# multimodallearning/convexAdam

Measured on AMD Instinct MI355X. Metric: volume-pairs/sec (160x192x224 MIND convex+Adam(80it)), higher is better.
Workload: dtype f32

## Files before the change

### convexadam_amd/_lib.py

```python
import ctypes as C
import os
import threading

import torch

_HERE = os.path.dirname(os.path.abspath(__file__))
LIB_PATH = os.environ.get("CONVEXADAM_HIP_LIB") or os.path.join(_HERE, "csrc", "libconvexadam_hip.so")

ABI_VERSION = 2
CVX_OK, CVX_ERR_INVALID_ARG, CVX_ERR_WORKSPACE, CVX_ERR_LAUNCH, CVX_ERR_UNSUPPORTED = 0, -1, -2, -3, -4


class CvxError(RuntimeError):
    def __init__(self, code, msg):
        super().__init__("libconvexadam_hip error %d: %s" % (code, msg))
        self.code = code


class Smoother(C.Structure):
    _fields_ = [("kind", C.c_int), ("n_boxes", C.c_int), ("box_k", C.c_int * 4), ("gauss_w", C.c_float * 5)]


class CorrOpts(C.Structure):
    _fields_ = [("cost", C.c_int), ("n_box", C.c_int), ("fast", C.c_int), ("f16", C.c_int)]


class PairParams(C.Structure):
    _fields_ = [("H", C.c_int), ("W", C.c_int), ("D", C.c_int), ("mind_r", C.c_int), ("mind_d", C.c_int),
                ("lambda_weight", C.c_float), ("grid_sp", C.c_int), ("disp_hw", C.c_int), ("selected_niter", C.c_int),
                ("selected_smooth", C.c_int), ("grid_sp_adam", C.c_int), ("ic", C.c_int), ("n_feat", C.c_int),
                ("cost_scale", C.c_float), ("cost", C.c_int), ("n_box", C.c_int), ("n_spline_pools", C.c_int), ("corr_fast", C.c_int),
                ("fp16_storage", C.c_int), ("ctx", C.c_void_p), ("adam_fast", C.c_int), ("reserved_", C.c_int * 3)]


_vp, _i, _f, _sz, _i64 = C.c_void_p, C.c_int, C.c_float, C.c_size_t, C.c_int64

SIGNATURES = {
    "cvx_version": (_i, []),
    "cvx_last_error": (C.c_char_p, []),
    "cvx_device_count": (_i, []),
    "cvx_context_create": (_vp, []),
    "cvx_context_destroy": (None, [_vp]),
    "cvx_context_bind": (_vp, [_vp]),
    "cvx_context_set_option": (_i, [_vp, C.c_char_p, C.c_longlong]),
    "cvx_context_get_option": (C.c_longlong, [_vp, C.c_char_p]),
    "cvx_context_set_adam_sqrt_table": (_i, [_vp, _vp, _vp]),
    "cvx_context_set_mind_exp_table": (_i, [_vp, _vp, C.c_uint, C.c_uint, _vp]),
    "cvx_set_adam_sqrt_table": (_i, [_vp]),
    "cvx_set_mind_exp_table": (_i, [_vp, C.c_uint, C.c_uint]),
    "cvx_expf_f32": (_i, [_vp, _vp, _sz, _vp]),
    "cvx_set_option": (_i, [C.c_char_p, C.c_longlong]),
    "cvx_get_option": (C.c_longlong, [C.c_char_p]),
    "cvx_affine_base_host": (None, [_i, _vp]),
    "cvx_disp_mesh_host": (None, [_i, _vp]),
    "cvx_disp_mesh_f32": (_i, [_i, _vp, _vp]),
    "cvx_affine_base_f32": (_i, [_i, _vp, _vp]),
    "cvx_mindssc_workspace_bytes": (_sz, [_i] * 5),
    "cvx_mindssc_f32": (_i, [_vp, _i, _i, _i, _i, _i, _vp, _vp, _sz, _vp]),
    "cvx_mindssc_pooled_scratch_bytes": (_sz, [_i] * 7),
    "cvx_mindssc_pooled_f32": (_i, [_vp, _i, _i, _i, _i, _i, _i, _vp, _i, _vp, _vp, _sz, _vp, _sz, _vp, _vp]),
    "cvx_avgpool_f32": (_i, [_vp, _i, _i, _i, _i, _i, _vp, _vp]),
    "cvx_round_f16_f32": (_i, [_vp, _i64, _vp]),
    "cvx_pack_field_f64": (_i, [_vp, _i, _i, _i, _i, _vp, _vp]),
    "cvx_box_smooth_workspace_bytes": (_sz, [_i] * 5),
    "cvx_box_smooth_f32": (_i, [_vp, _i, _i, _i, _i, _i, _i, _vp, _vp, _sz, _vp]),
    "cvx_box_grow_f32": (_i, [_vp, _i, _i, _i, _i, _i, _vp, _vp]),
    "cvx_mask_erode_f32": (_i, [_vp, _i, _i, _i, _f, _vp, _vp]),
    "cvx_gather_f32": (_i, [_vp, _vp, _i64, _vp, _vp]),
    "cvx_select_f32": (_i, [_vp, _vp, _vp, _i64, _vp, _vp]),
    "cvx_label_histogram_i64": (_i, [_vp, _i64, _i, _vp, _vp]),
    "cvx_label_weights_host": (_i, [_vp, _vp, _i, _vp, _vp]),
    "cvx_label_features_f32": (_i, [_vp, _i64, _i, _vp, _vp, _f, _vp, _vp]),
    "cvx_correlate_workspace_bytes": (_sz, [_i] * 5),
    "cvx_correlate_ex_f32": (_i, [_vp, _vp, _i, _i, _i, _i, _i, _vp, _vp, _vp, _vp, _sz, _vp]),
    "cvx_correlate_f32": (_i, [_vp, _vp, _i, _i, _i, _i, _i, _vp, _vp, _vp, _sz, _vp]),
    "cvx_coupled_convex_workspace_bytes": (_sz, [_i] * 4),
    "cvx_coupled_convex_f32": (_i, [_vp, _vp, _vp, _i, _i, _i, _i, _vp, _vp, _sz, _vp]),
    "cvx_coupled_convex_f16": (_i, [_vp, _vp, _vp, _i, _i, _i, _i, _vp, _vp, _sz, _vp]),
    "cvx_inverse_consistency_workspace_bytes": (_sz, [_i] * 3),
    "cvx_inverse_consistency_f32": (_i, [_vp, _vp, _i, _i, _i, _i, _vp, _vp, _vp, _vp, _vp, _vp, _sz, _vp]),
    "cvx_resize_trilinear_f32": (_i, [_vp, _i, _i, _i, _i, _vp, _i, _i, _i, _vp]),
    "cvx_grid_sample_f32": (_i, [_vp, _i, _i, _i, _i, _vp, _i, _i, _i, _vp, _vp]),
    "cvx_adam_workspace_bytes": (_sz, [_i] * 4),
    "cvx_adam_run_f32": (_i, [_vp, _vp, _i, _i, _i, _i, _vp, _vp, _vp, _f, _i, _i, _f, _vp, _vp, _vp, _vp, _vp, _vp, _i,
                              _vp, _vp, _sz, _vp]),
    "cvx_smooth_workspace_bytes": (_sz, [_i] * 4),
    "cvx_smooth_f32": (_i, [_vp, _i, _i, _i, _i, C.POINTER(Smoother), _i, _vp, _vp, _sz, _vp]),
    "cvx_adam_run_smoother_f32": (_i, [_vp, _vp, _i, _i, _i, _i, _vp, _vp, _vp, _f, _i, _i, _f, _vp, _vp, _vp, _vp, _vp, _vp, _i,
                                       _vp, C.POINTER(Smoother), _vp, _sz, _vp]),
    "cvx_adam_run_ex_f32": (_i, [_vp, _vp, _i, _i, _i, _i, _vp, _vp, _vp, _f, _i, _i, _f, _vp, _vp, _vp, _vp, _vp, _vp, _i,
                                 _vp, C.POINTER(Smoother), _i, _vp, _sz, _vp]),
    "cvx_adam_run_fast_f32": (_i, [_vp, _vp, _i, _i, _i, _i, _vp, _vp, _vp, _f, _i, _i, _f, _vp, _vp, _vp, _vp, _vp, _vp, _i,
                                   _vp, _vp, _sz, _vp]),
    "cvx_adam_run_fast_all_f32": (_i, [_vp, _vp, _i, _i, _i, _i, _vp, _vp, _vp, _f, _i, _i, _f, _vp, _vp, _vp, _vp, _vp, _vp, _i,
                                       _vp, _vp, _sz, _vp]),
    "cvx_adam_run_mode_f32": (_i, [_vp, _vp, _i, _i, _i, _i, _vp, _vp, _vp, _f, _i, _i, _f, _vp, _vp, _vp, _vp, _vp, _vp, _i,
                                   _vp, C.POINTER(Smoother), _i, _vp, _sz, _vp]),
    "cvx_smooth_fast_f32": (_i, [_vp, _i, _i, _i, C.POINTER(Smoother), _i, _vp, _vp]),
    "cvx_box3_fast_f32": (_i, [_vp, _i, _i, _i, _vp, _vp]),
    "cvx_register_pair_workspace_bytes": (_sz, [C.POINTER(PairParams)]),
    "cvx_register_pair_f32": (_i, [_vp, _vp, _vp, _vp, C.POINTER(PairParams), _vp, _vp, _vp, _sz, _vp]),
    "cvx_register_pair_snapshots_workspace_bytes": (_sz, [_vp, _i, _vp, _i]),
    "cvx_register_pair_snapshots_f32": (_i, [_vp, _vp, _vp, _vp, _vp, _vp, _i, _vp, _i, _vp, _vp, _sz, _vp]),
    "cvx_register_pairs_f32": (_i, [_i, _vp, _vp, _vp, _vp, C.POINTER(PairParams), _vp, _vp, _vp, _sz, _i, _vp]),
    "cvx_last_pair_profile": (_i, [_vp, _vp, _i]),
    "cvx_set_profiling": (None, [_i]),
    "cvx_jacobian_det_f32": (_i, [_vp, _i, _i, _i, _i, _vp, _vp]),
    "cvx_jacobian_stats_f64": (_i, [_vp, _i64, _vp, _vp]),
    "cvx_warp_labels_nearest_f32": (_i, [_vp, _vp, _i, _i, _i, _vp, _vp, _vp, _vp, _vp]),
    "cvx_label_overlap_i64": (_i, [_vp, _vp, _i64, _i, _vp, _vp]),
    "cvx_map_coordinates_linear_f64": (_i, [_vp, _vp, _i, _i, _i, _vp, _vp]),
    "cvx_feature_transform_workspace_bytes": (_sz, [_i, _i, _i]),
    "cvx_feature_transform_i32": (_i, [_vp, _i, _i, _i, _vp, _vp, _sz, _vp]),
    "cvx_feature_flat_index_i64": (_i, [_vp, _i, _i, _i, _i, _i, _vp, _vp]),
    "cvx_label_mask_f32": (_i, [_vp, _i, _i, _i, _i, _i, _vp, _vp, _vp, _vp]),
    "cvx_label_mask_scaled_f32": (_i, [_vp, _i, _i, _i, _i, _i, _i, _i, _f, _vp, _vp, _vp, _vp]),
    "cvx_edt_sqdist_i32": (_i, [_vp, _vp, _i, _i, _i, _vp, _vp]),
    "cvx_surface_hist_i64": (_i, [_vp, _vp, _vp, _i64, _i, _vp, _vp, _vp]),
    "cvx_hist_order_stats_i64": (_i, [_vp, _i, _i64, _i64, _vp, _vp]),
    "cvx_hist_percentile_neighbours_i64": (_i, [_vp, _i, _f, _vp, _vp]),
    "cvx_surface_hist_batch_i64": (_i, [_vp, _i, _i64, _i, _vp, _vp, _vp]),
    "cvx_hist_percentile_neighbours_batch_i64": (_i, [_vp, _i, _i, _f, _vp, _vp]),
    "cvx_edt_squared_workspace_bytes": (_sz, [_i, _i, _i, _i]),
    "cvx_edt_squared_i32": (_i, [_vp, _i, _i, _i, _i, _vp, _vp, _sz, _vp]),
    "cvx_edt_squared_labels_i32": (_i, [_vp, _i, _i, _i, _vp, _i, _vp, _vp, _sz, _vp]),
    "cvx_label_bits_bytes": (_sz, [_i, _i, _i, _i]),
    "cvx_label_bits_u64": (_i, [_vp, _i, _i, _i, _i, _vp, _vp]),
    "cvx_surface_distance_hist_i64": (_i, [_vp, _vp, _i, _i, _i, _i, _vp, _i, _vp, _i64, _vp, _i, _i, _vp]),
    "cvx_surface_distance_hist_bits_workspace_bytes": (_sz, [_i, _i, _i, _i]),
    "cvx_surface_distance_hist_bits_i64": (_i, [_vp, _vp, _i, _i, _i, _i, _vp, _i, _vp, _i64, _vp, _i, _i, _vp, _sz, _vp]),
    "cvx_tps_fit_workspace_bytes": (_sz, [_i, _i]),
    "cvx_tps_fit_f32": (_i, [_vp, _vp, _i, _i, _f, _vp, _vp, _sz, _vp]),
    "cvx_tps_eval_f32": (_i, [_vp, _i64, _vp, _vp, _i, _i, _vp, _vp]),
    "cvx_tps_dense_f32": (_i, [_i, _i, _i, _vp, _vp, _i, _i, _vp, _vp]),
    "cvx_resize_trilinear_ac_f32": (_i, [_vp, _i, _i, _i, _i, _vp, _i, _i, _i, _vp]),
}

_lib = None
_lock = threading.Lock()


def lib():
    global _lib
    if _lib is None:
        with _lock:
            if _lib is None:
                if not os.path.exists(LIB_PATH):
                    raise RuntimeError("%s not found: build it with `python -m convexadam_amd.csrc.build` "
                                       "(there is no CPU fallback)" % LIB_PATH)
                L = C.CDLL(LIB_PATH)
                for name, (res, args) in SIGNATURES.items():
                    fn = getattr(L, name)
                    fn.restype = res
                    fn.argtypes = args
                if L.cvx_version() != ABI_VERSION:
                    raise RuntimeError("%s reports ABI version %d, this binding needs %d (struct layouts differ): rebuild with "
                                       "`python -m convexadam_amd.csrc.build`" % (LIB_PATH, L.cvx_version(), ABI_VERSION))
                _lib = L
    return _lib


def check(rc):
    if rc != CVX_OK:
        raise CvxError(rc, lib().cvx_last_error().decode("utf-8", "replace"))


def require_device_tensor(t, name):
    if not isinstance(t, torch.Tensor):
        raise TypeError("%s must be a torch.Tensor" % name)
    if t.device.type != "cuda":
        raise RuntimeError("%s lives on %s: the convexadam_amd operators run only on a HIP (ROCm 'cuda') device; "
                           "there is no CPU path" % (name, t.device))
    return t


def f32c(t):
    return t.detach().to(torch.float32).contiguous()


def ptr(t):
    return C.c_void_p(t.data_ptr()) if t is not None else C.c_void_p(0)


def stream_ptr(device=None):
    return C.c_void_p(torch.cuda.current_stream(device).cuda_stream)


_tls = threading.local()


def workspace(nbytes, device):
    ws = getattr(_tls, "workspaces", None)
    if ws is None:
        ws = _tls.workspaces = {}
    key = (str(device), torch.cuda.current_stream(device).cuda_stream)
    buf = ws.get(key)
    if buf is None or buf.numel() < nbytes:
        ws[key] = buf = torch.empty(int(nbytes * 1.05) + 4096, dtype=torch.uint8, device=device)
    return buf


def release_workspaces():
    if getattr(_tls, "workspaces", None):
        _tls.workspaces.clear()
```

### convexadam_amd/csrc/adam.hip

```cpp
#include <math.h>

#include "cvx_common.h"

namespace cvx {

constexpr int BT_Z = 8, BT_Y = 8, BT_X = 32, BT_NT = 512, BT_PX = 48;

template <int PASS, bool BACKWARD, bool ADAM>
__device__ __forceinline__ void box_pass(const float* __restrict__ src, int sy, float* __restrict__ dst, int dz, int dy,
                                         int gz0, int gy0, int x0, int h, int w, int d, float* __restrict__ gout,
                                         float* __restrict__ P, float* __restrict__ m, float* __restrict__ v, AdamConsts ac,
                                         float* __restrict__ gsave) {
    constexpr int NP = 20 - PASS, C0 = 4 + PASS, SH = PASS - 1;
    const int nr = dz * dy * NP;
    for (int r = threadIdx.x; r < nr; r += BT_NT) {
        const int p = r % NP, row = r / NP;
        const int y = row % dy, z = row / dy;
        const int c = C0 + 2 * p;
        const float* win = src + ((z + 1) * sy + (y + 1)) * BT_PX + (c - 1 + SH);
        f32x2 s = {0.0f, 0.0f};
#pragma unroll
        for (int a = -1; a <= 1; ++a)
#pragma unroll
            for (int b = -1; b <= 1; ++b) {
                const float* q = win + (a * sy + b) * BT_PX;
                const f32x2 lo = lds_load2(q), hi = lds_load2(q + 2);
                s += lo;
                s.x += lo.y;
                s.y += hi.x;
                s += hi;
            }
        const int gz = gz0 + z, gy = gy0 + y, gx = x0 - 8 + c;
        const bool rowin = gz >= 0 && gz < h && gy >= 0 && gy < w;
        if (PASS < 3) {
            f32x2 o;
            o.x = (rowin && gx >= 0 && gx < d) ? div_exact<27>(s.x) : 0.0f;
            o.y = (rowin && gx + 1 >= 0 && gx + 1 < d) ? div_exact<27>(s.y) : 0.0f;
            lds_store2(dst + (z * dy + y) * BT_PX + (c + SH + 1), o);
        } else if (rowin) {
#pragma unroll
            for (int j = 0; j < 2; ++j) {
                const int cc = c + j;
                if (cc < 8 || cc > 39 || gx + j >= d) continue;
                const size_t i = ((size_t)gz * w + gy) * d + gx + j;
                const float sj = j ? s.y : s.x;
                if (!BACKWARD) gout[i] = div_exact<27>(sj);
                else if (!ADAM) gout[i] = sj;
                else {
                    const float g = sj;
                    const float mo = m[i];
                    const float mm = __builtin_fmaf(ac.w1, g - mo, mo);
                    float vv = v[i] * ac.b2;
                    vv = __builtin_fmaf(ac.omb2 * g, g, vv);
                    const float den = fdiv(adam_sqrt(vv, ac.sqrt_tbl), ac.bc2s) + 1e-8f;
                    P[i] = P[i] + fdiv(ac.neg_step * mm, den);
                    m[i] = mm;
                    v[i] = vv;
                    if (gsave) gsave[i] = g;
                }
            }
        }
    }
}

template <bool BACKWARD, bool ADAM>
__global__ __launch_bounds__(BT_NT) void k_box3x3(const float* __restrict__ in, float* __restrict__ out, int h, int w, int d,
                                                  float* __restrict__ P, float* __restrict__ m, float* __restrict__ v,
                                                  AdamConsts ac, float* __restrict__ gsave) {
    __shared__ __attribute__((aligned(16))) float A[(BT_Z + 6) * (BT_Y + 6) * BT_PX];
    __shared__ __attribute__((aligned(16))) float B[(BT_Z + 4) * (BT_Y + 4) * BT_PX];
    const int ntx = (d + BT_X - 1) / BT_X, nty = (w + BT_Y - 1) / BT_Y, ntz = (h + BT_Z - 1) / BT_Z;
    int b = blockIdx.x;
    const int tx = b % ntx; b /= ntx;
    const int ty = b % nty; b /= nty;
    const int tz = b % ntz; const int c = b / ntz;
    const int x0 = tx * BT_X, y0 = ty * BT_Y, z0 = tz * BT_Z;
    const size_t V = (size_t)h * w * d;
    const float* ic = in + (size_t)c * V;
    constexpr int AZ = BT_Z + 6, AY = BT_Y + 6, NCH = (BT_X + 8) / 4;
    const bool vec = (d & 3) == 0;
    for (int i = threadIdx.x; i < AZ * AY * NCH; i += BT_NT) {
        const int ch = i % NCH, y = (i / NCH) % AY, z = i / (NCH * AY);
        const int gz = z0 - 3 + z, gy = y0 - 3 + y, gx = x0 - 4 + 4 * ch;
        float4 q = make_float4(0.f, 0.f, 0.f, 0.f);
        if (gz >= 0 && gz < h && gy >= 0 && gy < w) {
            const float* rowp = ic + ((size_t)gz * w + gy) * d;
            if (vec && gx >= 0 && gx + 3 < d) q = *reinterpret_cast<const float4*>(rowp + gx);
            else {
                if (gx >= 0 && gx < d) q.x = rowp[gx];
                if (gx + 1 >= 0 && gx + 1 < d) q.y = rowp[gx + 1];
                if (gx + 2 >= 0 && gx + 2 < d) q.z = rowp[gx + 2];
                if (gx + 3 >= 0 && gx + 3 < d) q.w = rowp[gx + 3];
            }
            if (BACKWARD) { q.x = fdiv(q.x, 27.0f); q.y = fdiv(q.y, 27.0f); q.z = fdiv(q.z, 27.0f); q.w = fdiv(q.w, 27.0f); }
        }
        *reinterpret_cast<float4*>(A + (z * AY + y) * BT_PX + 4 + 4 * ch) = q;
    }
    cvx_barrier();
    float* oc = out ? out + (size_t)c * V : nullptr;
    float* Pc = P ? P + (size_t)c * V : nullptr;
    float* mc = m ? m + (size_t)c * V : nullptr;
    float* vc = v ? v + (size_t)c * V : nullptr;
    float* gs = gsave ? gsave + (size_t)c * V : nullptr;
    box_pass<1, BACKWARD, ADAM>(A, AY, B, BT_Z + 4, BT_Y + 4, z0 - 2, y0 - 2, x0, h, w, d, nullptr, nullptr, nullptr, nullptr, ac, nullptr);
    cvx_barrier();
    box_pass<2, BACKWARD, ADAM>(B, BT_Y + 4, A, BT_Z + 2, BT_Y + 2, z0 - 1, y0 - 1, x0, h, w, d, nullptr, nullptr, nullptr, nullptr, ac, nullptr);
    cvx_barrier();
    box_pass<3, BACKWARD, ADAM>(A, BT_Y + 2, nullptr, BT_Z, BT_Y, z0, y0, x0, h, w, d, oc, Pc, mc, vc, ac, gs);
}

__global__ __launch_bounds__(256) void k_adam_update(const float* __restrict__ G, float* __restrict__ P, float* __restrict__ m,
                                                     float* __restrict__ v, size_t n, AdamConsts ac) {
    const size_t i = (size_t)blockIdx.x * blockDim.x + threadIdx.x;
    if (i >= n) return;
    const float g = G[i];
    const float mo = m[i];
    const float mm = __builtin_fmaf(ac.w1, g - mo, mo);
    float vv = v[i] * ac.b2;
    vv = __builtin_fmaf(ac.omb2 * g, g, vv);
    const float den = fdiv(adam_sqrt(vv, ac.sqrt_tbl), ac.bc2s) + 1e-8f;
    P[i] = P[i] + fdiv(ac.neg_step * mm, den);
    m[i] = mm;
    v[i] = vv;
}

static int launch_box3x3(const float* in, float* out, int h, int w, int d, bool backward, float* P, float* m, float* v,
                         AdamConsts ac, float* gsave, hipStream_t s) {
    const bool force_tiled = options().box_tiled != 0;
    if (!force_tiled && (backward ? (out || P) && box3_tile_supported(in, out, h, w, d, P, m, v, gsave) : box3_tile_fwd_supported(in, out, h, w, d))) {
        long long ft = backward ? options().box_bwd_tile : options().box_fwd_tile;
        if (ft < 0) ft = box3_march_supported(d) ? box3_tile_fwd_auto(h, w, d) : 2000;
        if (ft >= 1000) return launch_box3_tile(in, out, h, w, d, (int)ft, backward, P, m, v, ac, gsave, s);
    }
    if (!force_tiled && box3_march_supported(d)) return launch_box3_march(in, out, h, w, d, backward, P, m, v, ac, gsave, s);
    const int nb = cdiv(d, BT_X) * cdiv(w, BT_Y) * cdiv(h, BT_Z) * 3;
    if (!backward) hipLaunchKernelGGL((k_box3x3<false, false>), dim3(nb), dim3(BT_NT), 0, s, in, out, h, w, d, P, m, v, ac, gsave);
    else if (!P) hipLaunchKernelGGL((k_box3x3<true, false>), dim3(nb), dim3(BT_NT), 0, s, in, out, h, w, d, P, m, v, ac, gsave);
    else hipLaunchKernelGGL((k_box3x3<true, true>), dim3(nb), dim3(BT_NT), 0, s, in, out, h, w, d, P, m, v, ac, gsave);
    return check_last("box3x3");
}

}

using namespace cvx;

extern "C" size_t cvx_adam_workspace_bytes(int C, int h, int w, int d) {
    const size_t V = (size_t)h * w * d, CP = (size_t)(C + 3) / 4 * 4;
    return 3 * (256 + sizeof(float) * 3 * V) + 2 * (256 + sizeof(float) * CP * (V + 1)) + 256;
}

extern "C" int cvx_adam_run_f32(const float* F2, const float* M2, int C, int h, int w, int d, float* P, float* m, float* v,
                                float lambda_weight, int niter, int step0, float cost_scale, const float* base_h,
                                const float* base_w, const float* base_d, float* U, float* grad_out,
                                const int* snapshot_iters_host, int n_snap, float* snapshots, void* workspace,
                                size_t workspace_bytes, void* stream) {
    return cvx_adam_run_smoother_f32(F2, M2, C, h, w, d, P, m, v, lambda_weight, niter, step0, cost_scale, base_h, base_w, base_d, U,
                                     grad_out, snapshot_iters_host, n_snap, snapshots, nullptr, workspace, workspace_bytes, stream);
}

extern "C" int cvx_adam_run_smoother_f32(const float* F2, const float* M2, int C, int h, int w, int d, float* P, float* m, float* v,
                                         float lambda_weight, int niter, int step0, float cost_scale, const float* base_h,
                                         const float* base_w, const float* base_d, float* U, float* grad_out,
                                         const int* snapshot_iters_host, int n_snap, float* snapshots, const cvx_smoother* sm,
                                         void* workspace, size_t workspace_bytes, void* stream) {
    return cvx::adam_run_impl(F2, M2, C, h, w, d, P, m, v, lambda_weight, niter, step0, cost_scale, base_h, base_w, base_d, U, grad_out,
                              snapshot_iters_host, n_snap, snapshots, sm, true, false, 0, workspace, workspace_bytes, stream);
}

extern "C" int cvx_adam_run_fast_f32(const float* F2, const float* M2, int C, int h, int w, int d, float* P, float* m, float* v,
                                     float lambda_weight, int niter, int step0, float cost_scale, const float* base_h,
                                     const float* base_w, const float* base_d, float* U, float* grad_out,
                                     const int* snapshot_iters_host, int n_snap, float* snapshots, void* workspace,
                                     size_t workspace_bytes, void* stream) {
    return cvx::adam_run_impl(F2, M2, C, h, w, d, P, m, v, lambda_weight, niter, step0, cost_scale, base_h, base_w, base_d, U, grad_out,
                              snapshot_iters_host, n_snap, snapshots, nullptr, true, false, 1, workspace, workspace_bytes, stream);
}

extern "C" int cvx_adam_run_fast_all_f32(const float* F2, const float* M2, int C, int h, int w, int d, float* P, float* m, float* v,
                                         float lambda_weight, int niter, int step0, float cost_scale, const float* base_h,
                                         const float* base_w, const float* base_d, float* U, float* grad_out,
                                         const int* snapshot_iters_host, int n_snap, float* snapshots, void* workspace,
                                         size_t workspace_bytes, void* stream) {
    return cvx::adam_run_impl(F2, M2, C, h, w, d, P, m, v, lambda_weight, niter, step0, cost_scale, base_h, base_w, base_d, U, grad_out,
                              snapshot_iters_host, n_snap, snapshots, nullptr, true, false, 2, workspace, workspace_bytes, stream);
}

extern "C" int cvx_adam_run_mode_f32(const float* F2, const float* M2, int C, int h, int w, int d, float* P, float* m, float* v,
                                     float lambda_weight, int niter, int step0, float cost_scale, const float* base_h,
                                     const float* base_w, const float* base_d, float* U, float* grad_out,
                                     const int* snapshot_iters_host, int n_snap, float* snapshots, const cvx_smoother* sm, int mode,
                                     void* workspace, size_t workspace_bytes, void* stream) {
    CVX_REQUIRE((mode & ~16) >= 0 && (mode & ~16) <= 2, "cvx_adam_run_mode_f32: mode must be 0 (exact), 1 (fast) or 2 (fast_all), + 16 for half-precision feature records");
    return cvx::adam_run_impl(F2, M2, C, h, w, d, P, m, v, lambda_weight, niter, step0, cost_scale, base_h, base_w, base_d, U, grad_out,
                              snapshot_iters_host, n_snap, snapshots, sm, true, (mode & 16) != 0, mode & 3, workspace, workspace_bytes, stream);
}

extern "C" int cvx_smooth_fast_f32(const float* in, int h, int w, int d, const cvx_smoother* sm, int backward, float* out, void* stream) {
    CVX_REQUIRE(in && out && sm && h > 0 && w > 0 && d > 0, "cvx_smooth_fast_f32: bad arguments");
    CVX_REQUIRE(sm->kind == 0, "cvx_smooth_fast_f32: box chains only (a Gaussian is three short 1-D convolutions already: cvx_smooth_f32)");
    return cvx::launch_boxchain_fast(in, out, h, w, d, *sm, backward != 0, as_stream(stream));
}

extern "C" int cvx_box3_fast_f32(const float* in, int h, int w, int d, float* out, void* stream) {
    CVX_REQUIRE(in && out && in != out && h > 0 && w > 0 && d > 0, "cvx_box3_fast_f32: bad arguments");
    return cvx::launch_box3_fast(in, out, h, w, d, nullptr, nullptr, nullptr, 1.0, 1.0, nullptr, as_stream(stream));
}

extern "C" int cvx_adam_run_ex_f32(const float* F2, const float* M2, int C, int h, int w, int d, float* P, float* m, float* v,
                                   float lambda_weight, int niter, int step0, float cost_scale, const float* base_h,
                                   const float* base_w, const float* base_d, float* U, float* grad_out,
                                   const int* snapshot_iters_host, int n_snap, float* snapshots, const cvx_smoother* sm,
                                   int feature_storage, void* workspace, size_t workspace_bytes, void* stream) {
    CVX_REQUIRE(feature_storage == 0 || feature_storage == 1, "cvx_adam_run_ex_f32: feature_storage must be 0 (float32) or 1 (fp16)");
    return cvx::adam_run_impl(F2, M2, C, h, w, d, P, m, v, lambda_weight, niter, step0, cost_scale, base_h, base_w, base_d, U, grad_out,
                              snapshot_iters_host, n_snap, snapshots, sm, true, feature_storage == 1, 0, workspace, workspace_bytes, stream);
}

int cvx::adam_run_impl(const float* F2, const float* M2, int C, int h, int w, int d, float* P, float* m, float* v,
                       float lambda_weight, int niter, int step0, float cost_scale, const float* base_h, const float* base_w,
                       const float* base_d, float* U, float* grad_out, const int* snapshot_iters_host, int n_snap,
                       float* snapshots, const cvx_smoother* sm, bool keep_state, bool f16_features, int fast, void* workspace,
                       size_t workspace_bytes, void* stream, bool features_are_records) {
    CVX_REQUIRE(F2 && M2 && P && m && v && U && base_h && base_w && base_d, "cvx_adam_run_f32: null pointer");
    CVX_REQUIRE(C > 0 && h > 1 && w > 1 && d > 1, "cvx_adam_run_f32: bad extent C=%d %dx%dx%d", C, h, w, d);
    CVX_REQUIRE(niter >= 0 && step0 >= 0, "cvx_adam_run_f32: negative iteration count");
    CVX_REQUIRE(n_snap == 0 || (snapshot_iters_host && snapshots), "cvx_adam_run_f32: snapshot buffers missing");
    if (!workspace || workspace_bytes < cvx_adam_workspace_bytes(C, h, w, d))
        return fail(CVX_ERR_WORKSPACE, "cvx_adam_run_f32: workspace too small");
    hipStream_t s = as_stream(stream);
    const size_t V = (size_t)h * w * d;
    Carver cv(workspace, workspace_bytes);
    float* gU = cv.take<float>(3 * V);
    float* t1 = cv.take<float>(3 * V);
    float* t2 = cv.take<float>(3 * V);
    const bool fused = !sm || (sm->kind == 0 && sm->n_boxes == 3 && sm->box_k[0] == 3 && sm->box_k[1] == 3 && sm->box_k[2] == 3);
    if (sm) {
        CVX_REQUIRE(sm->kind == 0 || sm->kind == 1, "cvx_adam_run_smoother_f32: smoother kind must be 0 or 1");
        if (sm->kind == 0) {
            CVX_REQUIRE(sm->n_boxes >= 1 && sm->n_boxes <= 4, "cvx_adam_run_smoother_f32: n_boxes must be 1..4");
            for (int i = 0; i < sm->n_boxes; ++i) CVX_REQUIRE(sm->box_k[i] >= 1 && (sm->box_k[i] & 1), "cvx_adam_run_smoother_f32: box size must be odd");
        }
    }
    if (fast && !fused && sm->kind == 0 && !boxchain_fast_supported(*sm, h, w, d))
        return fail(CVX_ERR_UNSUPPORTED, "adam_mode fast: box chain outside the separable kernel's range (odd sizes <= 9, lines of at most 320 voxels)");
    const int CP = (C + 3) / 4 * 4;
    float* Fcl = cv.take<float>((size_t)CP * (V + 1));
    float* Mcl = cv.take<float>((size_t)CP * (V + 1));
    if (features_are_records) { Fcl = const_cast<float*>(F2); Mcl = const_cast<float*>(M2); }
    else if (niter > 0) {
        int rc;
        if ((rc = launch_to_chunked(F2, C, V, Fcl, f16_features, s)) || (rc = launch_to_chunked(M2, C, V, Mcl, f16_features, s))) return rc;
    }

    const float nH = (float)((int64_t)3 * (h - 1) * w * d), nW = (float)((int64_t)3 * h * (w - 1) * d),
                nD = (float)((int64_t)3 * h * w * (d - 1));
    const float cH = lambda_weight / nH, cW = lambda_weight / nW, cD = lambda_weight / nD;
    const float gsc = ((1.0f / (float)V) * cost_scale) / (float)C;
    int snap = 0;
    for (int it = 0; it < niter; ++it) {
        int rc;
        const int step = step0 + it + 1;
        const double beta1 = 0.9, beta2 = 0.999;
        const double bc1 = 1.0 - pow(beta1, (double)step), bc2 = 1.0 - pow(beta2, (double)step);
        const AdamConsts ac = {(float)(1.0 - beta1), (float)beta2, (float)(1.0 - beta2), (float)sqrt(bc2), (float)(-(1.0 / bc1)), adam_sqrt_table()};
        if (fast == 2 && fused) { if ((rc = launch_box3_fast(P, U, h, w, d, nullptr, nullptr, nullptr, 1.0, 1.0, nullptr, s))) return rc; }
        else if (fast == 2 && sm->kind == 0) { if ((rc = launch_boxchain_fast(P, U, h, w, d, *sm, false, s))) return rc; }
        else if (fused) { if ((rc = launch_box3x3(P, U, h, w, d, false, nullptr, nullptr, nullptr, ac, nullptr, s))) return rc; }
        else if ((rc = launch_smoother(P, U, t1, 3, h, w, d, *sm, false, s))) return rc;
        profile_mark_kernel("adam.forward_boxes", s);
        const bool last = it == niter - 1;
        if (!(last && !keep_state && !grad_out)) {
        float* gsave = (grad_out && it == niter - 1) ? grad_out : nullptr;
        if (fast) {
            if ((rc = launch_warp_grad_fast(Fcl, Mcl, C, h, w, d, U, base_h, base_w, base_d, gsc, cH, cW, cD, gU, f16_features, s))) return rc;
            profile_mark_kernel("adam.warp_gradient", s);
            if (fused) { if ((rc = launch_box3_fast(gU, nullptr, h, w, d, P, m, v, bc1, bc2, gsave, s))) return rc; }
            else {
                if (sm->kind == 0) { if ((rc = launch_boxchain_fast(gU, t2, h, w, d, *sm, true, s))) return rc; }
                else if ((rc = launch_smoother(gU, t2, t1, 3, h, w, d, *sm, true, s))) return rc;
                if ((rc = launch_adam_update_fast(t2, P, m, v, 3 * V, bc1, bc2, s))) return rc;
                if (gsave) (void)hipMemcpyAsync(gsave, t2, sizeof(float) * 3 * V, hipMemcpyDeviceToDevice, s);
            }
        } else {
        if ((rc = launch_warp_grad(Fcl, Mcl, C, h, w, d, U, base_h, base_w, base_d, gsc, cH, cW, cD, gU, f16_features, s))) return rc;
        profile_mark_kernel("adam.warp_gradient", s);
        if (fused) { if ((rc = launch_box3x3(gU, nullptr, h, w, d, true, P, m, v, ac, gsave, s))) return rc; }
        else {
            if ((rc = launch_smoother(gU, t2, t1, 3, h, w, d, *sm, true, s))) return rc;
            hipLaunchKernelGGL(k_adam_update, dim3((unsigned)cdiv64((int64_t)(3 * V), 256)), dim3(256), 0, s, t2, P, m, v, 3 * V, ac);
            if (gsave) (void)hipMemcpyAsync(gsave, t2, sizeof(float) * 3 * V, hipMemcpyDeviceToDevice, s);
        }
        }
        }
        if (!(last && !keep_state && !grad_out)) profile_mark_kernel("adam.adjoint_update", s);
        while (snap < n_snap && snapshot_iters_host[snap] == it + 1) {
            (void)hipMemcpyAsync(snapshots + (size_t)snap * 3 * V, U, sizeof(float) * 3 * V, hipMemcpyDeviceToDevice, s);
            ++snap;
        }
    }
    return check_last("adam_run");
}
```

### convexadam_amd/csrc/api.hip

```cpp
#include <math.h>
#include <stdlib.h>
#include <string.h>
#include <new>

#include "cvx_common.h"

namespace cvx {

static thread_local char g_err[512] = "";

void set_error(const char* fmt, ...) {
    va_list ap;
    va_start(ap, fmt);
    vsnprintf(g_err, sizeof(g_err), fmt, ap);
    va_end(ap);
}
int fail(int code, const char* fmt, ...) {
    va_list ap;
    va_start(ap, fmt);
    vsnprintf(g_err, sizeof(g_err), fmt, ap);
    va_end(ap);
    return code;
}
int check_last(const char* what) {
    hipError_t e = hipGetLastError();
    if (e != hipSuccess) return fail(CVX_ERR_LAUNCH, "%s: %s", what, hipGetErrorString(e));
    return CVX_OK;
}

static long long env_ll(const char* name, long long dflt) {
    const char* e = getenv(name);
    return e ? atoll(e) : dflt;
}

}
struct cvx_context {
    cvx::Options opt;
    unsigned* sqrt_tbl = nullptr;
    unsigned char* exp_tbl = nullptr;
    unsigned exp_first = 0, exp_count = 0;
    int tbl_device = -1;
};
namespace cvx {
static Options env_options() {
    return {env_ll("CVX_MIND_TILED", 0),   env_ll("CVX_MIND_OVERLAP", 0),  env_ll("CVX_MM_TX", 0),        env_ll("CVX_MM_SLOTS", 512),          env_ll("CVX_BOX_TILED", 0),
            env_ll("CVX_NO_PRUNE", 0),     env_ll("CVX_CORR_UNFUSED", 0), env_ll("CVX_CORR_FUSED_ALL", 0), env_ll("CVX_PRUNE_STREAM_ABOVE", -1), env_ll("CVX_CF_CENSUS", 0), env_ll("CVX_CF_PRIO", 136),
            env_ll("CVX_WARP_FLAT", 0),    env_ll("CVX_BOX_YT", 8),       env_ll("CVX_BOX_WG_TARGET", 0),
            env_ll("CVX_BOX_XSPLIT", -1),  env_ll("CVX_BOX_CPT", 4),      env_ll("CVX_BOX_UNEVEN", 200), env_ll("CVX_BOX_ADAM_ROLE", 0), env_ll("CVX_BOX_DPP", 0),      env_ll("CVX_BOX_PK", 0),       env_ll("CVX_BOX_PRIO", 0),     env_ll("CVX_LABEL_POW_BLOCK", 32), 0,                             env_ll("CVX_MIND_MEAN_THREADS", 0),
            env_ll("CVX_EDT_SEQUENTIAL", 0), env_ll("CVX_WARP_OCTANT", 4), env_ll("CVX_BOX_FWD_TILE", -1), env_ll("CVX_BOX_BWD_TILE", -1), env_ll("CVX_BOX_WALK", 1), env_ll("CVX_CORR_DUAL", 0), env_ll("CVX_PRUNE_REFINE", 1), env_ll("CVX_MIND_RECORDS", 1), env_ll("CVX_RESIZE_UP2", 1), env_ll("CVX_MIND_BLOCKED", 1), env_ll("CVX_CORR_CERT", 1), env_ll("CVX_CC_DEBUG", 0), env_ll("CVX_IC_FUSED", 0), env_ll("CVX_MIND_SINGLE", 0), env_ll("CVX_MS_ZLEN", 0), env_ll("CVX_CF_MAP", 1), env_ll("CVX_CERT_UNFUSED", 0), env_ll("CVX_FBOX_TILE", 0)};
}
static cvx_context& default_context() {
    static cvx_context c = [] { cvx_context d; d.opt = env_options(); return d; }();
    return c;
}
static thread_local cvx_context* t_bound = nullptr;
static cvx_context& current_context() { return t_bound ? *t_bound : default_context(); }
Options& options() { return current_context().opt; }
const unsigned* adam_sqrt_table() { return current_context().sqrt_tbl; }
ExpTable mind_exp_table() {
    const cvx_context& c = current_context();
    return {c.exp_tbl, c.exp_first, c.exp_tbl ? c.exp_count : 0u};
}
ContextScope::ContextScope(const cvx_context* c) : prev_(t_bound), active_(c != nullptr) {
    if (active_) t_bound = const_cast<cvx_context*>(c);
}
ContextScope::~ContextScope() {
    if (active_) t_bound = static_cast<cvx_context*>(prev_);
}

static void drop_table(cvx_context& c, void** slot) {
    if (!*slot) return;
    int cur = 0;
    (void)hipGetDevice(&cur);
    if (c.tbl_device >= 0 && c.tbl_device != cur) (void)hipSetDevice(c.tbl_device);
    (void)hipDeviceSynchronize();
    (void)hipFree(*slot);
    if (c.tbl_device >= 0 && c.tbl_device != cur) (void)hipSetDevice(cur);
    (void)hipGetLastError();
    *slot = nullptr;
}
static int adopt_table(cvx_context& c, const void* src, size_t bytes, void** slot, hipStream_t s, const char* what) {
    if (!src) { drop_table(c, slot); return CVX_OK; }
    int cur = 0;
    (void)hipGetDevice(&cur);
    const bool other_table = (slot == reinterpret_cast<void**>(&c.sqrt_tbl)) ? c.exp_tbl != nullptr : c.sqrt_tbl != nullptr;
    if (c.tbl_device >= 0 && c.tbl_device != cur && other_table)
        return fail(CVX_ERR_INVALID_ARG, "%s: the context already holds a table on device %d (current device %d)", what, c.tbl_device, cur);
    void* p = nullptr;
    if (hipMalloc(&p, bytes) != hipSuccess) { (void)hipGetLastError(); return fail(CVX_ERR_LAUNCH, "%s: cannot allocate %zu bytes for the table copy", what, bytes); }
    if (hipMemcpyAsync(p, src, bytes, hipMemcpyDeviceToDevice, s) != hipSuccess || hipStreamSynchronize(s) != hipSuccess) {
        (void)hipGetLastError(); (void)hipFree(p);
        return fail(CVX_ERR_LAUNCH, "%s: table copy failed", what);
    }
    drop_table(c, slot);
    c.tbl_device = cur;
    *slot = p;
    return CVX_OK;
}
constexpr size_t kSqrtTableBytes = ((size_t)(1u << 24) + (1u << 23)) / 4;

__global__ __launch_bounds__(256) void k_expf(const float* __restrict__ x, float* __restrict__ out, size_t n) {
    for (size_t i = (size_t)blockIdx.x * blockDim.x + threadIdx.x; i < n; i += (size_t)gridDim.x * blockDim.x) out[i] = cvx_expf(x[i]);
}
struct OptName { const char* name; long long Options::*field; };
static const OptName kOptNames[] = {{"mind_tiled", &Options::mind_tiled},     {"mind_overlap", &Options::mind_overlap},   {"mm_tx", &Options::mm_tx},
                                    {"mm_slots", &Options::mm_slots},         {"box_tiled", &Options::box_tiled},
                                    {"no_prune", &Options::no_prune},         {"corr_unfused", &Options::corr_unfused}, {"corr_fused_all", &Options::corr_fused_all},
                                    {"prune_stream_above", &Options::prune_stream_above}, {"cf_census", &Options::cf_census}, {"cf_prio", &Options::cf_prio},
                                    {"warp_flat", &Options::warp_flat},       {"box_yt", &Options::box_yt},             {"box_wg_target", &Options::box_wg_target},
                                    {"box_xsplit", &Options::box_xsplit},     {"box_cpt", &Options::box_cpt},           {"box_uneven", &Options::box_uneven},     {"box_adam_role", &Options::box_adam_role}, {"box_dpp", &Options::box_dpp},           {"box_pk", &Options::box_pk},             {"box_prio", &Options::box_prio},         {"label_pow_block", &Options::label_pow_block}, {"census_ptr", &Options::census_ptr},     {"mind_mean_threads", &Options::mind_mean_threads},
                                    {"edt_sequential", &Options::edt_sequential}, {"warp_octant", &Options::warp_octant}, {"box_fwd_tile", &Options::box_fwd_tile}, {"box_bwd_tile", &Options::box_bwd_tile}, {"box_walk", &Options::box_walk}, {"corr_dual", &Options::corr_dual}, {"prune_refine", &Options::prune_refine}, {"mind_records", &Options::mind_records}, {"resize_up2", &Options::resize_up2}, {"mind_blocked", &Options::mind_blocked}, {"corr_cert", &Options::corr_cert}, {"cc_debug", &Options::cc_debug}, {"ic_fused", &Options::ic_fused}, {"mind_single", &Options::mind_single}, {"ms_zlen", &Options::ms_zlen}, {"cf_map", &Options::cf_map}, {"cert_unfused", &Options::cert_unfused}, {"fbox_tile", &Options::fbox_tile}};

}

static int set_option_of(cvx_context& c, const char* name, long long value) {
    for (const auto& o : cvx::kOptNames)
        if (name && strcmp(name, o.name) == 0) {
            if (strcmp(name, "box_xsplit") == 0 && value > 32) return cvx::fail(CVX_ERR_INVALID_ARG, "box_xsplit %lld: at most 32 x tiles", value);
            c.opt.*(o.field) = value;
            return CVX_OK;
        }
    return cvx::fail(CVX_ERR_INVALID_ARG, "cvx_set_option: unknown option '%s'", name ? name : "(null)");
}
static long long get_option_of(const cvx_context& c, const char* name) {
    for (const auto& o : cvx::kOptNames)
        if (name && strcmp(name, o.name) == 0) return c.opt.*(o.field);
    return -1;
}

extern "C" cvx_context* cvx_context_create(void) {
    cvx_context* c = new (std::nothrow) cvx_context();
    if (!c) { cvx::set_error("cvx_context_create: out of memory"); return nullptr; }
    c->opt = cvx::default_context().opt;
    return c;
}
extern "C" void cvx_context_destroy(cvx_context* c) {
    if (!c) return;
    if (cvx::t_bound == c) cvx::t_bound = nullptr;
    cvx::drop_table(*c, reinterpret_cast<void**>(&c->sqrt_tbl));
    cvx::drop_table(*c, reinterpret_cast<void**>(&c->exp_tbl));
    delete c;
}
extern "C" cvx_context* cvx_context_bind(cvx_context* c) {
    cvx_context* prev = cvx::t_bound;
    cvx::t_bound = c;
    return prev;
}
extern "C" int cvx_context_set_option(cvx_context* c, const char* name, long long value) {
    return set_option_of(c ? *c : cvx::default_context(), name, value);
}
extern "C" long long cvx_context_get_option(const cvx_context* c, const char* name) {
    return get_option_of(c ? *c : cvx::default_context(), name);
}
extern "C" int cvx_context_set_adam_sqrt_table(cvx_context* c, const void* device_table, void* stream) {
    cvx_context& x = c ? *c : cvx::default_context();
    return cvx::adopt_table(x, device_table, cvx::kSqrtTableBytes, reinterpret_cast<void**>(&x.sqrt_tbl), cvx::as_stream(stream), "cvx_context_set_adam_sqrt_table");
}
extern "C" int cvx_context_set_mind_exp_table(cvx_context* c, const void* device_table, unsigned first_key, unsigned count, void* stream) {
    cvx_context& x = c ? *c : cvx::default_context();
    if (device_table && count == 0) return cvx::fail(CVX_ERR_INVALID_ARG, "cvx_context_set_mind_exp_table: empty table");
    const int rc = cvx::adopt_table(x, device_table, ((size_t)count + 3) / 4, reinterpret_cast<void**>(&x.exp_tbl), cvx::as_stream(stream), "cvx_context_set_mind_exp_table");
    x.exp_first = device_table && rc == CVX_OK ? first_key : 0u;
    x.exp_count = device_table && rc == CVX_OK ? count : 0u;
    return rc;
}

extern "C" int cvx_set_option(const char* name, long long value) { return set_option_of(cvx::default_context(), name, value); }
extern "C" long long cvx_get_option(const char* name) { return get_option_of(cvx::default_context(), name); }
extern "C" int cvx_set_adam_sqrt_table(const void* device_table) { return cvx_context_set_adam_sqrt_table(nullptr, device_table, nullptr); }
extern "C" int cvx_set_mind_exp_table(const void* device_table, unsigned first_key, unsigned count) {
    return cvx_context_set_mind_exp_table(nullptr, device_table, first_key, count, nullptr);
}
extern "C" int cvx_expf_f32(const float* x, float* out, size_t n, void* stream) {
    if (n == 0) return CVX_OK;
    if (!x || !out) return cvx::fail(CVX_ERR_INVALID_ARG, "cvx_expf_f32: null pointer");
    const size_t blocks = (n + 255) / 256;
    hipLaunchKernelGGL(cvx::k_expf, dim3((unsigned)(blocks < 65536 ? blocks : 65536)), dim3(256), 0, cvx::as_stream(stream), x, out, n);
    return cvx::check_last("expf");
}

extern "C" int cvx_version(void) { return CVX_ABI_VERSION; }
extern "C" const char* cvx_last_error(void) { return cvx::g_err; }
extern "C" int cvx_device_count(void) {
    int n = 0;
    if (hipGetDeviceCount(&n) != hipSuccess) { (void)hipGetLastError(); return 0; }
    return n;
}

static void linspace_pm1(int S, float* out) {
    if (S == 1) { out[0] = -1.0f; return; }
    const float step = (1.0f - (-1.0f)) / (float)(S - 1);
    const int half = S / 2;
    for (int i = 0; i < S; ++i)
        out[i] = (i < half) ? fmaf(step, (float)i, -1.0f) : fmaf(-step, (float)(S - 1 - i), 1.0f);
}
extern "C" void cvx_affine_base_host(int S, float* out_host) {
    linspace_pm1(S, out_host);
    for (int i = 0; i < S; ++i) out_host[i] = (out_host[i] * (float)(S - 1)) / (float)S;
}
extern "C" void cvx_disp_mesh_host(int disp_hw, float* out_host) {
    const int n = 2 * disp_hw + 1;
    float lin[1024];
    if (n == 1) lin[0] = 0.0f;
    else linspace_pm1(n, lin);
    const size_t K = (size_t)n * n * n;
    for (int a = 0; a < n; ++a)
        for (int b = 0; b < n; ++b)
            for (int c = 0; c < n; ++c) {
                const size_t k = ((size_t)a * n + b) * n + c;
                out_host[0 * K + k] = lin[c] * (float)disp_hw;
                out_host[1 * K + k] = lin[b] * (float)disp_hw;
                out_host[2 * K + k] = lin[a] * (float)disp_hw;
            }
}
```

### convexadam_amd/csrc/boxtile.hip

```cpp
#include "cvx_common.h"

namespace cvx {

namespace {

constexpr unsigned BT_OOB = 0x80000000u;

struct BTWin { float w[3][6]; };

template <bool F, bool M, bool P>
__device__ __forceinline__ void bt_accum(const BTWin& t, float (&mid)[4], float (&pre)[4], float (&fin)[4]) {
    float f[4], m[4], p[4];
#pragma unroll
    for (int j = 0; j < 4; ++j) { f[j] = mid[j]; m[j] = pre[j]; p[j] = 0.0f; }
#pragma unroll
    for (int i = 0; i < 3; ++i)
#pragma unroll
        for (int j = 0; j < 4; ++j) {
            if (F) { f[j] += t.w[i][j]; f[j] += t.w[i][j + 1]; f[j] += t.w[i][j + 2]; }
            if (M) { m[j] += t.w[i][j]; m[j] += t.w[i][j + 1]; m[j] += t.w[i][j + 2]; }
            if (P) { p[j] += t.w[i][j]; p[j] += t.w[i][j + 1]; p[j] += t.w[i][j + 2]; }
        }
#pragma unroll
    for (int j = 0; j < 4; ++j) { fin[j] = f[j]; mid[j] = m[j]; pre[j] = p[j]; }
}

template <typename Load, typename Prep, typename Emit>
__device__ __forceinline__ void bt_walk(int L, Load load, Prep prep, Emit emit) {
    float mid[4] = {0.f, 0.f, 0.f, 0.f}, pre[4] = {0.f, 0.f, 0.f, 0.f}, fin[4];
    BTWin A, B;
    load(0, A);
    load(1, B);
    prep(A);
    bt_accum<false, false, true>(A, mid, pre, fin);
    load(2, A);
    prep(B);
    bt_accum<false, true, true>(B, mid, pre, fin);
    int n = 2;
#pragma unroll 1
    for (; n + 1 < L; n += 2) {
        load(n + 1, B);
        prep(A);
        bt_accum<true, true, true>(A, mid, pre, fin);
        emit(n - 2, fin);
        load(n + 2, A);
        prep(B);
        bt_accum<true, true, true>(B, mid, pre, fin);
        emit(n - 1, fin);
    }
    if (n < L) {
        load(L, B);
        prep(A);
        bt_accum<true, true, true>(A, mid, pre, fin);
        emit(L - 3, fin);
        load(L + 1, A);
        prep(B);
        bt_accum<true, true, false>(B, mid, pre, fin);
        emit(L - 2, fin);
        prep(A);
        bt_accum<true, false, false>(A, mid, pre, fin);
        emit(L - 1, fin);
    } else {
        load(L + 1, B);
        prep(A);
        bt_accum<true, true, false>(A, mid, pre, fin);
        emit(L - 2, fin);
        prep(B);
        bt_accum<true, false, false>(B, mid, pre, fin);
        emit(L - 1, fin);
    }
}

}

template <int TZ, int TY, int TXQ, int NW, int WPS, bool BACKWARD, bool ADAM>
__global__ __launch_bounds__(64 * NW, WPS) void k_box3_tile(const float* __restrict__ in, float* __restrict__ out, int h, int w, int d,
                                                           int ntz, int nty, int ntx, int ntiles, int NS1, int NS2, int NS3, FastDiv dvz, FastDiv dvx, FastDiv dvy,
                                                           FastDiv dn1, FastDiv dn2, FastDiv dn3, float* __restrict__ P, float* __restrict__ m, float* __restrict__ v, AdamConsts ac,
                                                           float* __restrict__ gsave) {
    constexpr int TX = 4 * TXQ, RS = TX + 4;
    constexpr int Z1 = TZ + 4, Y1 = TY + 4, Z2 = TZ + 2, Y2 = TY + 2;
    constexpr int SLOTS = NW * 4;
    static_assert(TXQ + 2 <= 16, "a row of quads must fit 16 lanes");
    __shared__ __attribute__((aligned(16))) float S[Z1 * Y1 * RS + Z2 * Y2 * RS + 8];
    float* S1 = S;
    float* S2 = S + Z1 * Y1 * RS;
    const int per_xcd = (int)(gridDim.x >> 3);
    const int bid = __builtin_amdgcn_readfirstlane((int)blockIdx.x);
    const int b = (bid & 7) * per_xcd + (bid >> 3);
    if (b >= ntiles) return;
    const int b1 = fastdiv(b, dvz), b2 = fastdiv(b1, dvx), c = fastdiv(b2, dvy);
    const int tz = b - b1 * ntz, tx = b1 - b2 * ntx, ty = b2 - c * nty;
    const int x0 = tx * TX, y0 = ty * TY, z0 = tz * TZ;
    const size_t V = (size_t)h * w * d;
    const float* ic = in + (size_t)c * V;
    float* oc = out ? out + (size_t)c * V : nullptr;
    const __amdgpu_buffer_rsrc_t ir = __builtin_amdgcn_make_buffer_rsrc(const_cast<float*>(ic), 0, (int)(V * sizeof(float)), 0x00020000);
    const int tid = threadIdx.x, q = tid & 15, slot = tid >> 4;
    const int wd = w * d;

    for (int item = slot; item < Y1 * NS1; item += SLOTS) {
        const int r = item % Y1, sg = item / Y1;
        const int p0 = fastdiv(sg * Z1, dn1), L = fastdiv((sg + 1) * Z1, dn1) - p0;
        const int gy = y0 - 2 + r, gx = x0 - 4 + 4 * q;
        const bool qin = gx >= 0 && gx < d && q < TXQ + 2;
        unsigned ro[3];
#pragma unroll
        for (int i = 0; i < 3; ++i) {
            const int yy = gy - 1 + i;
            ro[i] = (qin && yy >= 0 && yy < w) ? (unsigned)(yy * d + gx) * 4u : BT_OOB;
        }
        const int zin0 = z0 - 3 + p0;
        auto load = [&](int n, BTWin& t) {
            const int z = zin0 + n;
            const bool zok = z >= 0 && z < h;
            const unsigned zo = (unsigned)(zok ? z : 0) * (unsigned)wd * 4u;
#pragma unroll
            for (int i = 0; i < 3; ++i) {
                const float4 a = buffer_load16(ir, (zok && ro[i] != BT_OOB) ? ro[i] + zo : BT_OOB, 0);
                t.w[i][1] = a.x; t.w[i][2] = a.y; t.w[i][3] = a.z; t.w[i][4] = a.w;
            }
        };
        auto prep = [&](BTWin& t) {
            if (BACKWARD) {
#pragma unroll
                for (int i = 0; i < 3; ++i)
#pragma unroll
                    for (int j = 1; j <= 4; ++j) t.w[i][j] = t.w[i][j] == 0.0f ? t.w[i][j] : div_exact<27>(t.w[i][j]);
            }
#pragma unroll
            for (int i = 0; i < 3; ++i) {
                t.w[i][0] = __int_as_float(__builtin_amdgcn_update_dpp(0, __float_as_int(t.w[i][4]), 0x111, 0xf, 0xf, true));
                t.w[i][5] = __int_as_float(__builtin_amdgcn_update_dpp(0, __float_as_int(t.w[i][1]), 0x101, 0xf, 0xf, true));
            }
        };
        const bool rowin = qin && gy >= 0 && gy < w;
        float* dst = S1 + (p0 * Y1 + r) * RS + 4 * q - 2;
        auto emit = [&](int k, const float (&fin)[4]) {
            const int z = z0 - 2 + p0 + k;
            const bool ok = rowin && z >= 0 && z < h;
            float o[4];
#pragma unroll
            for (int j = 0; j < 4; ++j) o[j] = ok ? div_exact<27>(fin[j]) : 0.0f;
            float* p = dst + k * (Y1 * RS);
            if (q > 0 && q < TXQ + 2) lds_store2(p, f32x2{o[0], o[1]});
            if (q < TXQ + 1) lds_store2(p + 2, f32x2{o[2], o[3]});
        };
        bt_walk(L, load, prep, emit);
    }
    cvx_barrier();

    for (int item = slot; item < Y2 * NS2; item += SLOTS) {
        const int r = item % Y2, sg = item / Y2;
        const int p0 = fastdiv(sg * Z2, dn2), L = fastdiv((sg + 1) * Z2, dn2) - p0;
        if (q < TXQ + 1) {
            const float* src = S1 + (p0 * Y1 + r) * RS + 4 * q;
            auto load = [&](int n, BTWin& t) {
#pragma unroll
                for (int i = 0; i < 3; ++i) {
                    const float* rp = src + (n * Y1 + i) * RS;
                    const f32x4 a = lds_load4(rp);
                    const f32x2 e = lds_load2(rp + 4);
                    t.w[i][0] = a.x; t.w[i][1] = a.y; t.w[i][2] = a.z; t.w[i][3] = a.w; t.w[i][4] = e.x; t.w[i][5] = e.y;
                }
            };
            const int gy = y0 - 1 + r, gx = x0 - 1 + 4 * q;
            const bool rowin = gy >= 0 && gy < w;
            bool xin[4];
#pragma unroll
            for (int j = 0; j < 4; ++j) xin[j] = rowin && gx + j >= 0 && gx + j < d;
            float* dst = S2 + (p0 * Y2 + r) * RS + 4 * q;
            auto emit = [&](int k, const float (&fin)[4]) {
                const int z = z0 - 1 + p0 + k;
                const bool zok = z >= 0 && z < h;
                f32x4 o;
                o.x = (zok && xin[0]) ? div_exact<27>(fin[0]) : 0.0f;
                o.y = (zok && xin[1]) ? div_exact<27>(fin[1]) : 0.0f;
                o.z = (zok && xin[2]) ? div_exact<27>(fin[2]) : 0.0f;
                o.w = (zok && xin[3]) ? div_exact<27>(fin[3]) : 0.0f;
                lds_store4(dst + k * (Y2 * RS), o);
            };
            bt_walk(L, load, [](BTWin&) {}, emit);
        }
    }
    cvx_barrier();

    for (int item = slot; item < TY * NS3; item += SLOTS) {
        const int r = item % TY, sg = item / TY;
        const int p0 = fastdiv(sg * TZ, dn3), L = fastdiv((sg + 1) * TZ, dn3) - p0;
        const int gy = y0 + r, gx = x0 + 4 * q;
        if (q < TXQ && gy < w && gx < d) {
            const float* src = S2 + (p0 * Y2 + r) * RS + 4 * q;
            auto load = [&](int n, BTWin& t) {
#pragma unroll
                for (int i = 0; i < 3; ++i) {
                    const float* rp = src + (n * Y2 + i) * RS;
                    const f32x4 a = lds_load4(rp);
                    const f32x2 e = lds_load2(rp + 4);
                    t.w[i][0] = a.x; t.w[i][1] = a.y; t.w[i][2] = a.z; t.w[i][3] = a.w; t.w[i][4] = e.x; t.w[i][5] = e.y;
                }
            };
            const size_t o0 = ((size_t)(z0 + p0) * w + gy) * d + gx;
            auto emit = [&](int k, const float (&fin)[4]) {
                if (z0 + p0 + k >= h) return;
                const size_t o = o0 + (size_t)k * wd;
                if (!BACKWARD) {
                    *reinterpret_cast<float4*>(oc + o) = make_float4(div_exact<27>(fin[0]), div_exact<27>(fin[1]), div_exact<27>(fin[2]), div_exact<27>(fin[3]));
                } else if (!ADAM) {
                    *reinterpret_cast<float4*>(oc + o) = make_float4(fin[0], fin[1], fin[2], fin[3]);
                } else {
                    float* Pc = P + (size_t)c * V + o; float* mc = m + (size_t)c * V + o; float* vc = v + (size_t)c * V + o;
                    const float4 p4 = *reinterpret_cast<const float4*>(Pc), m4 = *reinterpret_cast<const float4*>(mc), v4 = *reinterpret_cast<const float4*>(vc);
                    float pp[4] = {p4.x, p4.y, p4.z, p4.w}, mm[4] = {m4.x, m4.y, m4.z, m4.w}, vv[4] = {v4.x, v4.y, v4.z, v4.w};
#pragma unroll
                    for (int j = 0; j < 4; ++j) adam_update(fin[j], pp[j], mm[j], vv[j], ac);
                    *reinterpret_cast<float4*>(Pc) = make_float4(pp[0], pp[1], pp[2], pp[3]);
                    *reinterpret_cast<float4*>(mc) = make_float4(mm[0], mm[1], mm[2], mm[3]);
                    *reinterpret_cast<float4*>(vc) = make_float4(vv[0], vv[1], vv[2], vv[3]);
                    if (gsave) *reinterpret_cast<float4*>(gsave + (size_t)c * V + o) = make_float4(fin[0], fin[1], fin[2], fin[3]);
                }
            };
            bt_walk(L, load, [](BTWin&) {}, emit);
        }
    }
}

bool box3_tile_supported(const float* in, const float* out, int h, int w, int d, const float* P, const float* m, const float* v, const float* gsave) {
    auto al = [](const void* p) { return (reinterpret_cast<uintptr_t>(p) & 15) == 0; };
    return (d % 4 == 0) && al(in) && al(out) && al(P) && al(m) && al(v) && al(gsave) && in != out && (size_t)h * w * d * 4 < ((size_t)1 << 31);
}
bool box3_tile_fwd_supported(const float* in, const float* out, int h, int w, int d) { return out && box3_tile_supported(in, out, h, w, d, nullptr, nullptr, nullptr, nullptr); }

template <int TZ, int TY, int TXQ, int NW, int WPS>
static int launch_tile_t(const float* in, float* out, int h, int w, int d, int ns1, int ns2, int ns3, bool backward, float* P, float* m, float* v,
                         AdamConsts ac, float* gsave, hipStream_t s) {
    const int ntz = cdiv(h, TZ), nty = cdiv(w, TY), ntx = cdiv(d, 4 * TXQ);
    const int ntiles = 3 * ntz * nty * ntx;
    const unsigned nb = (unsigned)((ntiles + 7) / 8 * 8);
    auto clampns = [](int ns, int planes) { return ns < 1 ? 1 : (ns > planes / 2 ? planes / 2 : ns); };
    const int a1 = clampns(ns1, TZ + 4), a2 = clampns(ns2, TZ + 2), a3 = clampns(ns3, TZ);
#define CVX_BT_LAUNCH(B, A) hipLaunchKernelGGL((k_box3_tile<TZ, TY, TXQ, NW, WPS, B, A>), dim3(nb), dim3(64 * NW), 0, s, in, out, h, w, d, ntz, nty, ntx, ntiles, a1, a2, a3, fastdiv_make(ntz), fastdiv_make(ntx), fastdiv_make(nty), fastdiv_make(a1), fastdiv_make(a2), fastdiv_make(a3), P, m, v, ac, gsave)
    if (!backward) CVX_BT_LAUNCH(false, false);
    else if (!P) CVX_BT_LAUNCH(true, false);
    else CVX_BT_LAUNCH(true, true);
#undef CVX_BT_LAUNCH
    return check_last("box3_tile");
}

int launch_box3_tile(const float* in, float* out, int h, int w, int d, int variant, bool backward, float* P, float* m, float* v, AdamConsts ac,
                     float* gsave, hipStream_t s) {
    const int kind = variant / 1000, ns = variant % 1000;
    int ns1 = ns / 100, ns2 = (ns / 10) % 10, ns3 = ns % 10;
    if (kind == 1) {
        if (!ns) { ns1 = 5; ns2 = 3; ns3 = 4; }
        return launch_tile_t<12, 8, 14, 8, 4>(in, out, h, w, d, ns1, ns2, ns3, backward, P, m, v, ac, gsave, s);
    }
    if (!ns) { ns1 = 4; ns2 = 3; ns3 = 4; }
    return launch_tile_t<12, 16, 14, 16, 4>(in, out, h, w, d, ns1, ns2, ns3, backward, P, m, v, ac, gsave, s);
}
int launch_box3_tile_fwd(const float* in, float* out, int h, int w, int d, int variant, hipStream_t s) {
    return launch_box3_tile(in, out, h, w, d, variant, false, nullptr, nullptr, nullptr, AdamConsts{}, nullptr, s);
}

int box3_tile_fwd_auto(int h, int w, int d) {
    const int n2 = 3 * cdiv(h, 12) * cdiv(w, 16) * cdiv(d, 56);
    return n2 >= 192 ? 2000 : 0;
}

}
```

### convexadam_amd/csrc/cvx_common.h

```cpp
#pragma once
#include <hip/hip_runtime.h>
#include <stdint.h>
#include <stdio.h>
#include <stdarg.h>

#include <mutex>

#include "convexadam_hip.h"

namespace cvx {

void set_error(const char* fmt, ...);
int fail(int code, const char* fmt, ...);
int check_last(const char* what);

#define CVX_REQUIRE(cond, ...)                                      \
    do {                                                            \
        if (!(cond)) return ::cvx::fail(CVX_ERR_INVALID_ARG, __VA_ARGS__); \
    } while (0)

static inline hipStream_t as_stream(void* s) { return reinterpret_cast<hipStream_t>(s); }
static inline size_t align_up(size_t v, size_t a) { return (v + a - 1) / a * a; }
static inline int cdiv(int a, int b) { return (a + b - 1) / b; }
static inline int64_t cdiv64(int64_t a, int64_t b) { return (a + b - 1) / b; }

template <typename KernelT>
static inline void ensure_dynamic_lds(KernelT kernel, size_t bytes, size_t& granted) {
    static std::mutex mu;
    std::lock_guard<std::mutex> lock(mu);
    if (bytes > granted) {
        (void)hipFuncSetAttribute(reinterpret_cast<const void*>(kernel), hipFuncAttributeMaxDynamicSharedMemorySize, (int)bytes);
        (void)hipGetLastError();
        granted = bytes;
    }
}

struct Carver {
    char* base;
    size_t size, used;
    Carver(void* p, size_t n) : base(static_cast<char*>(p)), size(n), used(0) {}
    template <typename T>
    T* take(size_t count) {
        size_t off = align_up(used, 256);
        used = off + count * sizeof(T);
        return reinterpret_cast<T*>(base + off);
    }
    bool ok() const { return used <= size && (base != nullptr || used == 0); }
};
static inline size_t carve_size(size_t used, size_t bytes) { return align_up(used, 256) + bytes; }

struct Options {
    long long mind_tiled;
    long long mind_overlap;
    long long mm_tx;
    long long mm_slots;
    long long box_tiled;
    long long no_prune;
    long long corr_unfused;
    long long corr_fused_all;
    long long prune_stream_above;
    long long cf_census;
    long long cf_prio;
    long long warp_flat;
    long long box_yt;
    long long box_wg_target;
    long long box_xsplit;
    long long box_cpt;
    long long box_uneven;
    long long box_adam_role;
    long long box_dpp;
    long long box_pk;
    long long box_prio;
    long long label_pow_block;
    long long census_ptr;
    long long mind_mean_threads;
    long long edt_sequential;
    long long warp_octant;
    long long box_fwd_tile;
    long long box_bwd_tile;
    long long box_walk;
    long long corr_dual;
    long long prune_refine;
    long long mind_records;
    long long resize_up2;
    long long mind_blocked;
    long long corr_cert;
    long long cc_debug;
    long long ic_fused;
    long long mind_single;
    long long ms_zlen;
    long long cf_map;
    long long cert_unfused;
    long long fbox_tile;
};
Options& options();
const unsigned* adam_sqrt_table();
class ContextScope {
public:
    explicit ContextScope(const cvx_context* c);
    ~ContextScope();
    ContextScope(const ContextScope&) = delete;
    ContextScope& operator=(const ContextScope&) = delete;
private:
    void* prev_;
    bool active_;
};

#ifdef CVX_RACE_JITTER
__device__ __forceinline__ void cvx_jitter() {
    unsigned t = (unsigned)__builtin_amdgcn_s_memtime();
    t ^= (unsigned)__builtin_amdgcn_s_getreg((4 << 0) | (0 << 6) | (31 << 11)) * 2654435761u;
    t ^= t >> 13; t *= 0x9E3779B1u; t ^= t >> 15;
    const int n = (int)(t & 15);
    for (int i = 0; i < n; ++i) __builtin_amdgcn_s_sleep(1);
}
__device__ __forceinline__ void cvx_barrier() { cvx_jitter(); __syncthreads(); cvx_jitter(); }
#else
__device__ __forceinline__ void cvx_barrier() { __syncthreads(); }
#endif

__device__ __forceinline__ int clampi(int v, int lo, int hi) { return v < lo ? lo : (v > hi ? hi : v); }

__device__ __forceinline__ float fdiv(float a, float b) { return __fdiv_rn(a, b); }
__device__ __forceinline__ float fsqrt(float a) { return sqrtf(a); }

__device__ __forceinline__ float cvx_expf(float d) {
    const float R_LN2f = 1.442695040888963407359924681001892137426645954152985934135449406931f;
    const float L2Uf = 0.693145751953125f, L2Lf = 1.428606765330187045e-06f;
    const float qf = rintf(d * R_LN2f);
    const int q = (int)qf;
    float s = __builtin_fmaf(qf, -L2Uf, d);
    s = __builtin_fmaf(qf, -L2Lf, s);
    float u = 0.000198527617612853646278381f;
    u = __builtin_fmaf(u, s, 0.00139304355252534151077271f);
    u = __builtin_fmaf(u, s, 0.00833336077630519866943359f);
    u = __builtin_fmaf(u, s, 0.0416664853692054748535156f);
    u = __builtin_fmaf(u, s, 0.166666671633720397949219f);
    u = __builtin_fmaf(u, s, 0.5f);
    u = 1.0f + __builtin_fmaf(s * s, u, s);
    u = __builtin_ldexpf(u, q);
    if (d < -104.0f) u = 0.0f;
    if (d > 100.0f) u = __int_as_float(0x7f800000);
    return u;
}

struct ExpTable { const unsigned char* tbl; unsigned first, count; };
ExpTable mind_exp_table();

typedef float f32x4 __attribute__((ext_vector_type(4)));
typedef __attribute__((address_space(3))) f32x4 lds_f32x4;
__device__ __forceinline__ f32x4 lds_load4(const float* p) { return *(const volatile lds_f32x4*)p; }
__device__ __forceinline__ void lds_store4(float* p, f32x4 v) { *(volatile lds_f32x4*)p = v; }

typedef int i32x4 __attribute__((ext_vector_type(4)));
__device__ __forceinline__ float4 buffer_load16(__amdgpu_buffer_rsrc_t rsrc, unsigned lane_off, unsigned uni_off) {
    const i32x4 v = __builtin_bit_cast(i32x4, __builtin_amdgcn_raw_buffer_load_b128(rsrc, (int)lane_off, (int)uni_off, 0));
    return make_float4(__int_as_float(v.x), __int_as_float(v.y), __int_as_float(v.z), __int_as_float(v.w));
}

typedef float f32x2 __attribute__((ext_vector_type(2)));
typedef __attribute__((address_space(3))) f32x2 lds_f32x2;
__device__ __forceinline__ f32x2 lds_load2(const float* p) { return *(const volatile lds_f32x2*)p; }
__device__ __forceinline__ void lds_store2(float* p, f32x2 v) { *(volatile lds_f32x2*)p = v; }

template <int D>
__device__ __forceinline__ float div_exact(float x) {
    static_assert(D == 8 || D == 27 || D == 64 || D == 125 || D == 343, "divisor not verified");
    constexpr float r = 1.0f / (float)D;
    const float q = x * r;
    const float e = __builtin_fmaf(-(float)D, q, x);
    return __builtin_fmaf(e, r, q);
}

template <int N>
__device__ __forceinline__ float cascade_seq(const float (&v)[N]) {
    static_assert(N < 256, "two cascade levels");
    float a0 = 0.f, a1 = 0.f;
    int i = 0;
#pragma unroll
    for (; i + 16 <= N; i += 16) {
#pragma unroll
        for (int j = 0; j < 16; ++j) a0 += v[i + j];
        a1 += a0;
        a0 = 0.f;
    }
#pragma unroll
    for (; i < N; ++i) a0 += v[i];
    a0 += a1;
    return a0;
}
template <int N>
__device__ __forceinline__ float outer_sum_ilp(const float (&v)[N]) {
    static_assert(N / 4 < 16, "single cascade level inside the interleaved sums");
    float p[4] = {0.f, 0.f, 0.f, 0.f};
#pragma unroll
    for (int i = 0; i < N / 4; ++i)
#pragma unroll
        for (int k = 0; k < 4; ++k) p[k] += v[4 * i + k];
#pragma unroll
    for (int i = (N / 4) * 4; i < N; ++i) p[0] += v[i];
    p[0] += p[1];
    p[0] += p[2];
    p[0] += p[3];
    return p[0];
}

__device__ __forceinline__ unsigned long long pack_min_key(float v, unsigned idx) {
    unsigned b = __float_as_uint(v);
    b = (b & 0x80000000u) ? ~b : (b | 0x80000000u);
    if (v != v) b = 0u;
    return ((unsigned long long)b << 32) | idx;
}

struct Tri {
    float ix, iy, iz;
    int x0, y0, z0;
    float tnw, tne, tsw, tse, bnw, bne, bsw, bse;
};
__device__ __forceinline__ float unnormalize(float g, int S) { return ((g + 1.0f) * (float)S - 1.0f) * 0.5f; }
__device__ __forceinline__ void tri_setup(Tri& t, float gx, float gy, float gz, int h, int w, int d) {
    t.ix = unnormalize(gx, d);
    t.iy = unnormalize(gy, w);
    t.iz = unnormalize(gz, h);
    const float fx = floorf(t.ix), fy = floorf(t.iy), fz = floorf(t.iz);
    t.x0 = (int)fmaxf(fminf(fx, 1.0e9f), -1.0e9f);
    t.y0 = (int)fmaxf(fminf(fy, 1.0e9f), -1.0e9f);
    t.z0 = (int)fmaxf(fminf(fz, 1.0e9f), -1.0e9f);
    const float x1 = (float)(t.x0 + 1), y1 = (float)(t.y0 + 1), z1 = (float)(t.z0 + 1);
    const float x0f = (float)t.x0, y0f = (float)t.y0, z0f = (float)t.z0;
    t.tnw = (x1 - t.ix) * (y1 - t.iy) * (z1 - t.iz);
    t.tne = (t.ix - x0f) * (y1 - t.iy) * (z1 - t.iz);
    t.tsw = (x1 - t.ix) * (t.iy - y0f) * (z1 - t.iz);
    t.tse = (t.ix - x0f) * (t.iy - y0f) * (z1 - t.iz);
    t.bnw = (x1 - t.ix) * (y1 - t.iy) * (t.iz - z0f);
    t.bne = (t.ix - x0f) * (y1 - t.iy) * (t.iz - z0f);
    t.bsw = (x1 - t.ix) * (t.iy - y0f) * (t.iz - z0f);
    t.bse = (t.ix - x0f) * (t.iy - y0f) * (t.iz - z0f);
}
__device__ __forceinline__ bool inb3(int z, int y, int x, int h, int w, int d) {
    return z >= 0 && z < h && y >= 0 && y < w && x >= 0 && x < d;
}
__device__ __forceinline__ float tri_sample(const Tri& t, const float* __restrict__ vol, int h, int w, int d) {
    const int x0 = t.x0, y0 = t.y0, z0 = t.z0, x1 = x0 + 1, y1 = y0 + 1, z1 = z0 + 1;
    const bool zi0 = (unsigned)z0 < (unsigned)h, zi1 = (unsigned)z1 < (unsigned)h, yi0 = (unsigned)y0 < (unsigned)w,
               yi1 = (unsigned)y1 < (unsigned)w, xi0 = (unsigned)x0 < (unsigned)d, xi1 = (unsigned)x1 < (unsigned)d;
    const int zc0 = clampi(z0, 0, h - 1), zc1 = clampi(z1, 0, h - 1), yc0 = clampi(y0, 0, w - 1), yc1 = clampi(y1, 0, w - 1),
              xc0 = clampi(x0, 0, d - 1), xc1 = clampi(x1, 0, d - 1);
    const size_t r00 = ((size_t)zc0 * w + yc0) * d, r01 = ((size_t)zc0 * w + yc1) * d, r10 = ((size_t)zc1 * w + yc0) * d,
                 r11 = ((size_t)zc1 * w + yc1) * d;
    const float v0 = vol[r00 + xc0], v1 = vol[r00 + xc1], v2 = vol[r01 + xc0], v3 = vol[r01 + xc1], v4 = vol[r10 + xc0],
                v5 = vol[r10 + xc1], v6 = vol[r11 + xc0], v7 = vol[r11 + xc1];
    float o = 0.0f, n;
    n = o + v0 * t.tnw; o = (zi0 && yi0 && xi0) ? n : o;
    n = o + v1 * t.tne; o = (zi0 && yi0 && xi1) ? n : o;
    n = o + v2 * t.tsw; o = (zi0 && yi1 && xi0) ? n : o;
    n = o + v3 * t.tse; o = (zi0 && yi1 && xi1) ? n : o;
    n = o + v4 * t.bnw; o = (zi1 && yi0 && xi0) ? n : o;
    n = o + v5 * t.bne; o = (zi1 && yi0 && xi1) ? n : o;
    n = o + v6 * t.bsw; o = (zi1 && yi1 && xi0) ? n : o;
    n = o + v7 * t.bse; o = (zi1 && yi1 && xi1) ? n : o;
    return o;
}

struct FastDiv { unsigned d, m; };
static inline FastDiv fastdiv_make(int d) { FastDiv f; f.d = (unsigned)d; f.m = d <= 1 ? 0u : (unsigned)((((unsigned long long)1 << 32) + (unsigned)d - 1) / (unsigned)d); return f; }
__device__ __forceinline__ int fastdiv(int n, FastDiv f) { return f.d <= 1 ? n : (int)__umulhi((unsigned)n, f.m); }

void profile_mark_kernel(const char* name, hipStream_t s);

int launch_box_zero(const float* in, float* out, int C, int H, int W, int D, int k, bool backward, hipStream_t s);
int launch_smoother(const float* in, float* out, float* tmp, int C, int H, int W, int D, const cvx_smoother& sm, bool backward,
                    hipStream_t s);
int launch_argmin_keys(const void* ssd, bool f16, int K, size_t v, unsigned long long* keys, bool arm, hipStream_t s);
int* coupled_ws_counts(void* workspace, size_t workspace_bytes, int h, int w, int d, int disp_hw);
int launch_argmin(const void* ssd, bool f16, const float* mesh, const float* u, float coef, bool coupled, int K, size_t v,
                  unsigned long long* keys, int64_t* argmin_out, hipStream_t s);
int launch_resize(const float* in, int C, int h, int w, int d, float* out, int H, int W, int D, float pre_mul,
                  float post_div, hipStream_t s);
int launch_resize2(const float* in, int C, int h, int w, int d, int H, int W, int D, float* scratch, float* out, int h2, int w2,
                   int d2, float post_div, hipStream_t s);
struct AdamConsts { float w1, b2, omb2, bc2s, neg_step; const unsigned* sqrt_tbl; };
__device__ __forceinline__ float adam_sqrt(float x, const unsigned* __restrict__ tbl) {
    float r = fsqrt(x);
    if (tbl) {
        const unsigned b = __float_as_uint(x), e = b >> 23, mant = b & 0x7fffffu;
        if (b != 0 && e < 255) {
            const unsigned key = e ? (((e & 1u) << 23) | mant) : ((1u << 24) | mant);
            const unsigned code = (tbl[key >> 4] >> ((key & 15u) * 2u)) & 3u;
            if (code) r = __uint_as_float(__float_as_uint(r) + (code == 1u ? 1u : 0xffffffffu));
        }
    }
    return r;
}
__device__ __forceinline__ bool argmin_better(float cost, float best) { return (cost < best) | ((cost != cost) & (best == best)); }
__device__ __forceinline__ void adam_update(float g, float& P, float& m, float& v, const AdamConsts& ac) {
    const float mm = __builtin_fmaf(ac.w1, g - m, m);
    float vv = v * ac.b2;
    vv = __builtin_fmaf(ac.omb2 * g, g, vv);
    const float den = fdiv(adam_sqrt(vv, ac.sqrt_tbl), ac.bc2s) + 1e-8f;
    P = P + fdiv(ac.neg_step * mm, den);
    m = mm;
    v = vv;
}
int adam_run_impl(const float* F2, const float* M2, int C, int h, int w, int d, float* P, float* m, float* v, float lambda_weight,
                  int niter, int step0, float cost_scale, const float* base_h, const float* base_w, const float* base_d, float* U,
                  float* grad_out, const int* snapshot_iters_host, int n_snap, float* snapshots, const cvx_smoother* sm,
                  bool keep_state, bool f16_features, int fast, void* workspace, size_t workspace_bytes, void* stream,
                  bool features_are_records = false);
int coupled_convex_impl(const void* ssd, bool f16, const int64_t* argmin, const float* mesh, int h, int w, int d, int disp_hw, float* out,
                        bool argmin_is_exact, void* workspace, size_t workspace_bytes, void* stream);
int coupled_convex_dual_impl(const void* ssdA, const int64_t* argminA, float* outA, void* wsA, const void* ssdB, bool f16, const int64_t* argminB,
                             float* outB, void* wsB, const float* mesh, int h, int w, int d, int disp_hw, size_t workspace_bytes,
                             void* stream, bool counts_zeroed = false);
bool mind_pooled_supported(int H, int W, int D, int g1, int g2);
int launch_mind_pooled(const float* img, int H, int W, int D, int radius, int dilation, int g1, float* out1, int g2, float* out2,
                       float* raw, void* workspace, size_t workspace_bytes, hipStream_t s, int records = 0);
bool mind_pooled_records_supported(int H, int W, int D, int g1, int g2);
size_t mind_pooled_raw_floats(int H, int W, int D, int g1, int g2);
bool corr_box2_supported(int h, int w, int d, int px);
int launch_corr_box2(const float* raw, int K, int h, int w, int d, int px, float* ssd, hipStream_t s, bool fast = false);
bool corr_fused_supported(int C, int h, int w, int d, int hw);
void corr_fused_set_prep_hook(void (*hook)(hipStream_t));
int corr_fused_items(int C, int h, int w, int d, int hw);
bool corr_fused_tiled(int C, int h, int w, int d, int hw);
void corr_call_prep_hook(hipStream_t s);
bool corr_certfast_pays(int C, int h, int w, int d, int hw);
size_t corr_fused_workspace_bytes(int C, int h, int w, int d, int hw);
int launch_corr_fused(const float* fix, const float* mov, int C, int h, int w, int d, int hw, int cost, int n_box, int fast, int f16,
                      void* ssd, void* workspace, size_t workspace_bytes, hipStream_t s);
int launch_corr_fused_dual(const float* fix, const float* mov, int C, int h, int w, int d, int hw, int cost, int n_box, int fast, int f16,
                           void* ssd, void* ssd_rev, void* workspace, size_t workspace_bytes, void* workspace_rev, hipStream_t s);
bool corr_cert_supported(int C, int h, int w, int d, int hw);
size_t corr_cert_workspace_bytes(int C, int h, int w, int d, int hw);
int launch_corr_cert(const float* fix, const float* mov, int C, int h, int w, int d, int hw, float* ssdu, void* workspace, size_t workspace_bytes,
                     hipStream_t s);
bool corr_certfast_supported(int C, int h, int w, int d, int hw);
size_t corr_certfast_workspace_bytes(int C, int h, int w, int d, int hw);
int launch_corr_certfast(const float* fix, const float* mov, int C, int h, int w, int d, int hw, float* ssdu, void* workspace, size_t workspace_bytes,
                         hipStream_t s);
size_t corr_certify_workspace_bytes(int C, int h, int w, int d, int hw, bool plain = false);
int corr_certified_argmin(const float* ssdu, const float* fix, const float* mov, int C, int h, int w, int d, int hw, int64_t* argmin,
                          void* workspace, size_t workspace_bytes, hipStream_t s);
int coupled_convex_cert_impl(const float* ssduA, const float* fixA, const float* movA, float* outA, void* wsA, const float* ssduB, const float* fixB,
                             const float* movB, float* outB, void* wsB, const float* mesh, int C, int h, int w, int d, int hw, size_t workspace_bytes,
                             hipStream_t s, int stage = 0);
bool corr_use_unfused(int C, int h, int w, int d, int hw, bool variant);
bool box3_march_supported(int d);
int launch_box3_march(const float* in, float* out, int h, int w, int d, bool backward, float* P, float* m, float* v,
                      AdamConsts ac, float* gsave, hipStream_t s);
bool box3_tile_fwd_supported(const float* in, const float* out, int h, int w, int d);
int launch_box3_tile_fwd(const float* in, float* out, int h, int w, int d, int variant, hipStream_t s);
int box3_tile_fwd_auto(int h, int w, int d);
bool box3_tile_supported(const float* in, const float* out, int h, int w, int d, const float* P, const float* m, const float* v, const float* gsave);
int launch_box3_tile(const float* in, float* out, int h, int w, int d, int variant, bool backward, float* P, float* m, float* v, AdamConsts ac,
                     float* gsave, hipStream_t s);
int launch_to_chunked(const float* in, int C, size_t V, float* out, bool half, hipStream_t s);
int launch_warp_grad(const float* Fcl, const float* Mcl, int C, int h, int w, int d, const float* U, const float* bh,
                     const float* bw, const float* bd, float gsc, float cH, float cW, float cD, float* gU, bool half, hipStream_t s);
int launch_warp_grad_fast(const float* Fcl, const float* Mcl, int C, int h, int w, int d, const float* U, const float* bh,
                          const float* bw, const float* bd, float gsc, float cH, float cW, float cD, float* gU, bool half, hipStream_t s);
int launch_box3_fast(const float* in, float* out, int h, int w, int d, float* P, float* m, float* v, double bc1, double bc2,
                     float* gsave, hipStream_t s);
bool boxchain_fast_supported(const cvx_smoother& sm, int h, int w, int d);
int launch_boxchain_fast(const float* in, float* out, int h, int w, int d, const cvx_smoother& sm, bool reverse, hipStream_t s);
int launch_adam_update_fast(const float* G, float* P, float* m, float* v, size_t n, double bc1, double bc2, hipStream_t s);

}
```

### convexadam_amd/csrc/warp.hip

```cpp
#include "cvx_common.h"

namespace cvx {

__global__ __launch_bounds__(256) void k_to_chunked(const float* __restrict__ in, int C, size_t V, float* __restrict__ out) {
    const size_t p = (size_t)blockIdx.x * blockDim.x + threadIdx.x;
    if (p > V) return;
    const int c0 = 4 * (int)blockIdx.y;
    float4 r = make_float4(0.f, 0.f, 0.f, 0.f);
    if (p < V) {
        const float* src = in + (size_t)c0 * V + p;
        r.x = src[0];
        if (c0 + 1 < C) r.y = src[V];
        if (c0 + 2 < C) r.z = src[2 * V];
        if (c0 + 3 < C) r.w = src[3 * V];
    }
    reinterpret_cast<float4*>(out)[(size_t)blockIdx.y * (V + 1) + p] = r;
}

typedef _Float16 h16x4 __attribute__((ext_vector_type(4)));
__global__ __launch_bounds__(256) void k_to_chunked_h(const float* __restrict__ in, int C, size_t V, uint2* __restrict__ out) {
    const size_t p = (size_t)blockIdx.x * blockDim.x + threadIdx.x;
    if (p > V) return;
    const int c0 = 4 * (int)blockIdx.y;
    float4 r = make_float4(0.f, 0.f, 0.f, 0.f);
    if (p < V) {
        const float* src = in + (size_t)c0 * V + p;
        r.x = src[0];
        if (c0 + 1 < C) r.y = src[V];
        if (c0 + 2 < C) r.z = src[2 * V];
        if (c0 + 3 < C) r.w = src[3 * V];
    }
    const h16x4 o = {(_Float16)r.x, (_Float16)r.y, (_Float16)r.z, (_Float16)r.w};
    out[(size_t)blockIdx.y * (V + 1) + p] = __builtin_bit_cast(uint2, o);
}
__device__ __forceinline__ float4 buffer_load8h(__amdgpu_buffer_rsrc_t rsrc, unsigned lane_off, unsigned uni_off) {
    const h16x4 v = __builtin_bit_cast(h16x4, __builtin_amdgcn_raw_buffer_load_b64(rsrc, (int)lane_off, (int)uni_off, 0));
    return make_float4((float)v.x, (float)v.y, (float)v.z, (float)v.w);
}

template <bool BUF, bool HALF = false>
__global__ __launch_bounds__(256) void k_warp_grad(const float* __restrict__ F2, const float* __restrict__ M2, int C, int CP,
                                                   int h, int w, int d, const float* __restrict__ U,
                                                   const float* __restrict__ bh, const float* __restrict__ bw,
                                                   const float* __restrict__ bd, float gsc, float cH, float cW, float cD,
                                                   float* __restrict__ gU, unsigned long long* __restrict__ census, FastDiv dx, FastDiv dy,
                                                   float sc0, float sc1, float sc2) {
    const size_t V = (size_t)h * w * d;
    if (census && threadIdx.x == 0) {
        census[4 * blockIdx.x] = __builtin_amdgcn_s_memrealtime();
        census[4 * blockIdx.x + 3] = __builtin_amdgcn_s_getreg((4 << 0) | (0 << 6) | (31 << 11)) | ((unsigned long long)__builtin_amdgcn_s_getreg((20 << 0) | (0 << 6) | (31 << 11)) << 32);
    }
    const int ntx = (d + 15) / 16, nty = (w + 3) / 4, ntz = (h + 3) / 4;
    const int per_xcd = (int)(gridDim.x >> 3);
    const int bid = __builtin_amdgcn_readfirstlane((int)blockIdx.x);
    const int tile = (bid & 7) * per_xcd + (bid >> 3);
    if (tile >= ntx * nty * ntz) return;
    const int trow = fastdiv(tile, dx), tbz = fastdiv(trow, dy);
    const int tbx = tile - trow * ntx, tby = trow - tbz * nty;
    const int x = tbx * 16 + (threadIdx.x & 15), y = tby * 4 + ((threadIdx.x >> 4) & 3), z = tbz * 4 + (threadIdx.x >> 6);
    if (x >= d || y >= w || z >= h) return;
    const unsigned p = (unsigned)((z * w + y) * d + x);
    const float uH = U[p], uW = U[V + p], uD = U[2 * V + p];
    Tri t;
    tri_setup(t, bd[x] + fdiv(uD, sc2), bw[y] + fdiv(uW, sc1), bh[z] + fdiv(uH, sc0), h, w, d);
    const int x0 = t.x0, y0 = t.y0, z0 = t.z0, x1 = x0 + 1, y1 = y0 + 1, z1 = z0 + 1;
    const float fx0 = (float)x0, fy0 = (float)y0, fz0 = (float)z0, fx1 = (float)x1, fy1 = (float)y1, fz1 = (float)z1;
    const bool zin0 = (unsigned)z0 < (unsigned)h, zin1 = (unsigned)z1 < (unsigned)h, yin0 = (unsigned)y0 < (unsigned)w,
               yin1 = (unsigned)y1 < (unsigned)w, xin0 = (unsigned)x0 < (unsigned)d, xin1 = (unsigned)x1 < (unsigned)d;
    const int r00 = (z0 * w + y0) * d, r01 = (z0 * w + y1) * d, r10 = (z1 * w + y0) * d, r11 = (z1 * w + y1) * d;
    constexpr unsigned REC = HALF ? 8u : 16u;
    const unsigned zero_rec = (unsigned)V * REC;
    unsigned off[8];
    off[0] = (zin0 && yin0 && xin0) ? (unsigned)(r00 + x0) * REC : zero_rec; off[1] = (zin0 && yin0 && xin1) ? (unsigned)(r00 + x1) * REC : zero_rec;
    off[2] = (zin0 && yin1 && xin0) ? (unsigned)(r01 + x0) * REC : zero_rec; off[3] = (zin0 && yin1 && xin1) ? (unsigned)(r01 + x1) * REC : zero_rec;
    off[4] = (zin1 && yin0 && xin0) ? (unsigned)(r10 + x0) * REC : zero_rec; off[5] = (zin1 && yin0 && xin1) ? (unsigned)(r10 + x1) * REC : zero_rec;
    off[6] = (zin1 && yin1 && xin0) ? (unsigned)(r11 + x0) * REC : zero_rec; off[7] = (zin1 && yin1 && xin1) ? (unsigned)(r11 + x1) * REC : zero_rec;
    const float wgt[8] = {t.tnw, t.tne, t.tsw, t.tse, t.bnw, t.bne, t.bsw, t.bse};
    const float ax[8] = {fy1 - t.iy, fy1 - t.iy, t.iy - fy0, t.iy - fy0, fy1 - t.iy, fy1 - t.iy, t.iy - fy0, t.iy - fy0};
    const float bx[8] = {fz1 - t.iz, fz1 - t.iz, fz1 - t.iz, fz1 - t.iz, t.iz - fz0, t.iz - fz0, t.iz - fz0, t.iz - fz0};
    const float ay[8] = {fx1 - t.ix, t.ix - fx0, fx1 - t.ix, t.ix - fx0, fx1 - t.ix, t.ix - fx0, fx1 - t.ix, t.ix - fx0};
    const float bz[8] = {fy1 - t.iy, fy1 - t.iy, t.iy - fy0, t.iy - fy0, fy1 - t.iy, fy1 - t.iy, t.iy - fy0, t.iy - fy0};
    float gix = 0.f, giy = 0.f, giz = 0.f;
    const unsigned foff = p * REC;
    const unsigned chunk_bytes = (unsigned)(V + 1) * REC;
    const __amdgpu_buffer_rsrc_t mr = __builtin_amdgcn_make_buffer_rsrc(const_cast<float*>(M2), 0, (int)(chunk_bytes * (unsigned)(CP / 4)), 0x00020000);
    const __amdgpu_buffer_rsrc_t fr = __builtin_amdgcn_make_buffer_rsrc(const_cast<float*>(F2), 0, (int)(chunk_bytes * (unsigned)(CP / 4)), 0x00020000);
    unsigned coff = 0;
    for (int c0 = 0; c0 < CP / 4; ++c0, coff += chunk_bytes) {
        float vv[8][4], fv[4];
#pragma unroll
        for (int k = 0; k < 8; ++k) {
            const float4 q = HALF ? buffer_load8h(mr, off[k], coff) : BUF ? buffer_load16(mr, off[k], coff) : *reinterpret_cast<const float4*>(reinterpret_cast<const char*>(M2) + (size_t)c0 * chunk_bytes + off[k]);
            vv[k][0] = q.x; vv[k][1] = q.y; vv[k][2] = q.z; vv[k][3] = q.w;
        }
        const float4 fq = HALF ? buffer_load8h(fr, foff, coff) : BUF ? buffer_load16(fr, foff, coff) : *reinterpret_cast<const float4*>(reinterpret_cast<const char*>(F2) + (size_t)c0 * chunk_bytes + foff);
        fv[0] = fq.x; fv[1] = fq.y; fv[2] = fq.z; fv[3] = fq.w;
#pragma unroll
        for (int j = 0; j < 4; ++j) {
            float wv = 0.0f;
#pragma unroll
            for (int k = 0; k < 8; ++k) wv += vv[k][j] * wgt[k];
            const float df = wv - fv[j];
            const float gOut = gsc * (2.0f * df);
            gix -= vv[0][j] * ax[0] * bx[0] * gOut; giy -= vv[0][j] * ay[0] * bx[0] * gOut; giz -= vv[0][j] * ay[0] * bz[0] * gOut;
            gix += vv[1][j] * ax[1] * bx[1] * gOut; giy -= vv[1][j] * ay[1] * bx[1] * gOut; giz -= vv[1][j] * ay[1] * bz[1] * gOut;
            gix -= vv[2][j] * ax[2] * bx[2] * gOut; giy += vv[2][j] * ay[2] * bx[2] * gOut; giz -= vv[2][j] * ay[2] * bz[2] * gOut;
            gix += vv[3][j] * ax[3] * bx[3] * gOut; giy += vv[3][j] * ay[3] * bx[3] * gOut; giz -= vv[3][j] * ay[3] * bz[3] * gOut;
            gix -= vv[4][j] * ax[4] * bx[4] * gOut; giy -= vv[4][j] * ay[4] * bx[4] * gOut; giz += vv[4][j] * ay[4] * bz[4] * gOut;
            gix += vv[5][j] * ax[5] * bx[5] * gOut; giy -= vv[5][j] * ay[5] * bx[5] * gOut; giz += vv[5][j] * ay[5] * bz[5] * gOut;
            gix -= vv[6][j] * ax[6] * bx[6] * gOut; giy += vv[6][j] * ay[6] * bx[6] * gOut; giz += vv[6][j] * ay[6] * bz[6] * gOut;
            gix += vv[7][j] * ax[7] * bx[7] * gOut; giy += vv[7][j] * ay[7] * bx[7] * gOut; giz += vv[7][j] * ay[7] * bz[7] * gOut;
        }
    }
    float g[3];
    g[0] = fdiv(((float)h / 2.0f) * giz, sc0);
    g[1] = fdiv(((float)w / 2.0f) * giy, sc1);
    g[2] = fdiv(((float)d / 2.0f) * gix, sc2);
    const unsigned sH = (unsigned)(w * d);
    const unsigned pxp = x < d - 1 ? p + 1 : p, pxm = x > 0 ? p - 1 : p, pzp = z < h - 1 ? p + sH : p, pzm = z > 0 ? p - sH : p,
                   pyp = y < w - 1 ? p + (unsigned)d : p, pym = y > 0 ? p - (unsigned)d : p;
    float nb[3][6];
    const __amdgpu_buffer_rsrc_t ur = __builtin_amdgcn_make_buffer_rsrc(const_cast<float*>(U), 0, (int)(12u * (unsigned)V), 0x00020000);
    const unsigned nboff[6] = {4u * pxp, 4u * pxm, 4u * pzp, 4u * pzm, 4u * pyp, 4u * pym};
#pragma unroll
    for (int a = 0; a < 3; ++a)
#pragma unroll
        for (int k = 0; k < 6; ++k) nb[a][k] = __builtin_bit_cast(float, __builtin_amdgcn_raw_buffer_load_b32(ur, (int)nboff[k], (int)(4u * (unsigned)V) * a, 0));
    const float uc3[3] = {uH, uW, uD};
#pragma unroll
    for (int a = 0; a < 3; ++a) {
        const float uc = uc3[a];
        float acc = g[a], t;
        t = acc + -(cD * (2.0f * (nb[a][0] - uc))); acc = x < d - 1 ? t : acc;
        t = acc +  (cD * (2.0f * (uc - nb[a][1]))); acc = x > 0 ? t : acc;
        t = acc + -(cH * (2.0f * (nb[a][2] - uc))); acc = z < h - 1 ? t : acc;
        t = acc +  (cH * (2.0f * (uc - nb[a][3]))); acc = z > 0 ? t : acc;
        t = acc + -(cW * (2.0f * (nb[a][4] - uc))); acc = y < w - 1 ? t : acc;
        t = acc +  (cW * (2.0f * (uc - nb[a][5]))); acc = y > 0 ? t : acc;
        (gU + (size_t)a * V)[p] = acc;
    }
    if (census && threadIdx.x == 0) census[4 * blockIdx.x + 2] = __builtin_amdgcn_s_memrealtime();
}


int launch_to_chunked(const float* in, int C, size_t V, float* out, bool half, hipStream_t s) {
    const int CP = (C + 3) / 4 * 4;
    if ((size_t)(CP / 4) * (V + 1) * 16 >= ((size_t)1 << 31)) return fail(CVX_ERR_UNSUPPORTED, "adam_run: control grid too large (%zu voxels x %d channels)", V, C);
    if (half) hipLaunchKernelGGL(k_to_chunked_h, dim3((unsigned)cdiv64((int64_t)(V + 1), 256), CP / 4), dim3(256), 0, s, in, C, V, reinterpret_cast<uint2*>(out));
    else hipLaunchKernelGGL(k_to_chunked, dim3((unsigned)cdiv64((int64_t)(V + 1), 256), CP / 4), dim3(256), 0, s, in, C, V, out);
    return check_last("to_chunked");
}

int launch_warp_grad(const float* Fcl, const float* Mcl, int C, int h, int w, int d, const float* U, const float* bh,
                     const float* bw, const float* bd, float gsc, float cH, float cW, float cD, float* gU, bool half, hipStream_t s) {
    const int CP = (C + 3) / 4 * 4;
    const dim3 gv((unsigned)((cdiv(d, 16) * cdiv(w, 4) * cdiv(h, 4) + 7) / 8 * 8));
    unsigned long long* census = reinterpret_cast<unsigned long long*>(options().census_ptr);
    if (census) census += 8 * 1024;
    const FastDiv dx = fastdiv_make(cdiv(d, 16)), dy = fastdiv_make(cdiv(w, 4));
    const float sc0 = (float)((h - 1) / 2.0), sc1 = (float)((w - 1) / 2.0), sc2 = (float)((d - 1) / 2.0);
    if (half) hipLaunchKernelGGL((k_warp_grad<true, true>), gv, dim3(256), 0, s, Fcl, Mcl, C, CP, h, w, d, U, bh, bw, bd, gsc, cH, cW, cD, gU, census, dx, dy, sc0, sc1, sc2);
    else if (options().warp_flat) hipLaunchKernelGGL(k_warp_grad<false>, gv, dim3(256), 0, s, Fcl, Mcl, C, CP, h, w, d, U, bh, bw, bd, gsc, cH, cW, cD, gU, census, dx, dy, sc0, sc1, sc2);
    else hipLaunchKernelGGL(k_warp_grad<true>, gv, dim3(256), 0, s, Fcl, Mcl, C, CP, h, w, d, U, bh, bw, bd, gsc, cH, cW, cD, gU, census, dx, dy, sc0, sc1, sc2);
    return check_last("warp_grad");
}

}
```

### include/convexadam_hip.h

```cpp
#ifndef CONVEXADAM_HIP_H
#define CONVEXADAM_HIP_H

#include <stddef.h>
#include <stdint.h>

#ifdef __cplusplus
extern "C" {
#endif

#pragma GCC visibility push(default)

#define CVX_OK 0
#define CVX_ERR_INVALID_ARG (-1)
#define CVX_ERR_WORKSPACE (-2)
#define CVX_ERR_LAUNCH (-3)
#define CVX_ERR_UNSUPPORTED (-4)
#define CVX_MAX_DISP_HW 15

#define CVX_ABI_VERSION 2
int cvx_version(void);
const char* cvx_last_error(void);
int cvx_device_count(void);

typedef struct cvx_context cvx_context;
cvx_context* cvx_context_create(void);
void cvx_context_destroy(cvx_context* ctx);
cvx_context* cvx_context_bind(cvx_context* ctx);
int cvx_context_set_option(cvx_context* ctx, const char* name, long long value);
long long cvx_context_get_option(const cvx_context* ctx, const char* name);
int cvx_set_option(const char* name, long long value);
long long cvx_get_option(const char* name);

void cvx_affine_base_host(int S, float* out_host);
void cvx_disp_mesh_host(int disp_hw, float* out_host);
int cvx_disp_mesh_f32(int disp_hw, float* out_device, void* stream);
int cvx_affine_base_f32(int S, float* out_device, void* stream);

size_t cvx_mindssc_workspace_bytes(int H, int W, int D, int radius, int dilation);
int cvx_mindssc_f32(const float* img, int H, int W, int D, int radius, int dilation, float* out,
                    void* workspace, size_t workspace_bytes, void* stream);

size_t cvx_mindssc_pooled_scratch_bytes(int H, int W, int D, int radius, int dilation, int g1, int g2);
int cvx_mindssc_pooled_f32(const float* img, int H, int W, int D, int radius, int dilation, int g1, float* out1, int g2, float* out2,
                           void* scratch, size_t scratch_bytes, void* workspace, size_t workspace_bytes, int* repaired_host, void* stream);

int cvx_avgpool_f32(const float* in, int C, int H, int W, int D, int g, float* out, void* stream);

int cvx_round_f16_f32(float* x, int64_t n, void* stream);

size_t cvx_box_smooth_workspace_bytes(int C, int H, int W, int D, int passes);
int cvx_box_smooth_f32(const float* in, int C, int H, int W, int D, int k, int passes, float* out,
                       void* workspace, size_t workspace_bytes, void* stream);
int cvx_box_grow_f32(const float* in, int C, int H, int W, int D, int k, float* out, void* stream);

int cvx_pack_field_f64(const float* field, int H, int W, int D, int quantize, double* out, void* stream);

int cvx_mask_erode_f32(const float* mask, int H, int W, int D, float threshold, float* out, void* stream);
int cvx_gather_f32(const float* src, const int64_t* index, int64_t n, float* out, void* stream);
int cvx_select_f32(const float* mask, const float* a, const float* b, int64_t n, float* out, void* stream);

int cvx_label_histogram_i64(const float* lab, int64_t V, int max_label, int64_t* hist ,
                            void* stream);
int cvx_label_weights_host(const int64_t* hist_fix_host, const int64_t* hist_mov_host, int max_label,
                           int* present_host, float* weights_host);
int cvx_label_features_f32(const float* lab, int64_t V, int C, const int* present ,
                           const float* weights , float mult, float* feat, void* stream);

size_t cvx_correlate_workspace_bytes(int C, int h, int w, int d, int disp_hw);
int cvx_correlate_f32(const float* fix, const float* mov, int C, int h, int w, int d, int disp_hw,
                      float* ssd, int64_t* argmin, void* workspace, size_t workspace_bytes, void* stream);
typedef struct cvx_corr_opts { int cost, n_box, fast, f16; } cvx_corr_opts;
int cvx_correlate_ex_f32(const float* fix, const float* mov, int C, int h, int w, int d, int disp_hw, const cvx_corr_opts* opts,
                         float* ssd, int64_t* argmin, void* workspace, size_t workspace_bytes, void* stream);

size_t cvx_coupled_convex_workspace_bytes(int h, int w, int d, int disp_hw);
int cvx_coupled_convex_f32(const float* ssd, const int64_t* argmin, const float* mesh, int h, int w, int d,
                           int disp_hw, float* out, void* workspace, size_t workspace_bytes, void* stream);

int cvx_coupled_convex_f16(const void* ssd_half, const int64_t* argmin, const float* mesh, int h, int w, int d,
                           int disp_hw, float* out, void* workspace, size_t workspace_bytes, void* stream);

size_t cvx_inverse_consistency_workspace_bytes(int h, int w, int d);
int cvx_inverse_consistency_f32(const float* f1, const float* f2, int h, int w, int d, int iters,
                                const float* base_h, const float* base_w, const float* base_d, float* o1,
                                float* o2, void* workspace, size_t workspace_bytes, void* stream);

int cvx_resize_trilinear_f32(const float* in, int C, int h, int w, int d, float* out, int H, int W, int D,
                             void* stream);

int cvx_grid_sample_f32(const float* vol, int C, int h, int w, int d, const float* grid, int ho, int wo, int dd,
                        float* out, void* stream);

typedef struct cvx_smoother {
    int kind;
    int n_boxes;
    int box_k[4];
    float gauss_w[5];
} cvx_smoother;
size_t cvx_smooth_workspace_bytes(int C, int H, int W, int D);
int cvx_smooth_f32(const float* in, int C, int H, int W, int D, const cvx_smoother* sm, int backward, float* out,
                   void* workspace, size_t workspace_bytes, void* stream);

size_t cvx_adam_workspace_bytes(int C, int h, int w, int d);
int cvx_adam_run_f32(const float* F2, const float* M2, int C, int h, int w, int d, float* P, float* m,
                     float* v, float lambda_weight, int niter, int step0, float cost_scale,
                     const float* base_h, const float* base_w, const float* base_d, float* U, float* grad_out,
                     const int* snapshot_iters_host, int n_snap, float* snapshots, void* workspace,
                     size_t workspace_bytes, void* stream);

int cvx_context_set_adam_sqrt_table(cvx_context* ctx, const void* device_table, void* stream);
int cvx_set_adam_sqrt_table(const void* device_table);

int cvx_context_set_mind_exp_table(cvx_context* ctx, const void* device_table, unsigned first_key, unsigned count, void* stream);
int cvx_set_mind_exp_table(const void* device_table, unsigned first_key, unsigned count);
int cvx_expf_f32(const float* x, float* out, size_t n, void* stream);

int cvx_adam_run_smoother_f32(const float* F2, const float* M2, int C, int h, int w, int d, float* P, float* m,
                              float* v, float lambda_weight, int niter, int step0, float cost_scale,
                              const float* base_h, const float* base_w, const float* base_d, float* U, float* grad_out,
                              const int* snapshot_iters_host, int n_snap, float* snapshots, const cvx_smoother* sm,
                              void* workspace, size_t workspace_bytes, void* stream);

int cvx_adam_run_ex_f32(const float* F2, const float* M2, int C, int h, int w, int d, float* P, float* m,
                        float* v, float lambda_weight, int niter, int step0, float cost_scale,
                        const float* base_h, const float* base_w, const float* base_d, float* U, float* grad_out,
                        const int* snapshot_iters_host, int n_snap, float* snapshots, const cvx_smoother* sm,
                        int feature_storage, void* workspace, size_t workspace_bytes, void* stream);

int cvx_adam_run_fast_f32(const float* F2, const float* M2, int C, int h, int w, int d, float* P, float* m,
                          float* v, float lambda_weight, int niter, int step0, float cost_scale,
                          const float* base_h, const float* base_w, const float* base_d, float* U, float* grad_out,
                          const int* snapshot_iters_host, int n_snap, float* snapshots,
                          void* workspace, size_t workspace_bytes, void* stream);
int cvx_adam_run_fast_all_f32(const float* F2, const float* M2, int C, int h, int w, int d, float* P, float* m,
                              float* v, float lambda_weight, int niter, int step0, float cost_scale,
                              const float* base_h, const float* base_w, const float* base_d, float* U, float* grad_out,
                              const int* snapshot_iters_host, int n_snap, float* snapshots,
                              void* workspace, size_t workspace_bytes, void* stream);
int cvx_adam_run_mode_f32(const float* F2, const float* M2, int C, int h, int w, int d, float* P, float* m,
                          float* v, float lambda_weight, int niter, int step0, float cost_scale,
                          const float* base_h, const float* base_w, const float* base_d, float* U, float* grad_out,
                          const int* snapshot_iters_host, int n_snap, float* snapshots, const cvx_smoother* sm, int mode,
                          void* workspace, size_t workspace_bytes, void* stream);
int cvx_smooth_fast_f32(const float* in, int h, int w, int d, const cvx_smoother* sm, int backward, float* out, void* stream);
int cvx_box3_fast_f32(const float* in, int h, int w, int d, float* out, void* stream);

typedef struct cvx_pair_params {
    int H, W, D;
    int mind_r, mind_d;
    float lambda_weight;
    int grid_sp, disp_hw;
    int selected_niter, selected_smooth;
    int grid_sp_adam;
    int ic;
    int n_feat;
    float cost_scale;
    int cost;
    int n_box;
    int n_spline_pools;
    int corr_fast;
    int fp16_storage;
    const cvx_context* ctx;
    int adam_fast;
    int reserved_[3];
} cvx_pair_params;

size_t cvx_register_pair_workspace_bytes(const cvx_pair_params* p);
int cvx_register_pair_f32(const float* img_fixed, const float* img_moving, const float* feat_fixed,
                          const float* feat_moving, const cvx_pair_params* p, float* out_field,
                          int* out_dims_host, void* workspace, size_t workspace_bytes, void* stream);

size_t cvx_register_pair_snapshots_workspace_bytes(const cvx_pair_params* p, int n_snap, const int* smooth_host, int n_smooth);
int cvx_register_pair_snapshots_f32(const float* img_fixed, const float* img_moving, const float* feat_fixed,
                                    const float* feat_moving, const cvx_pair_params* p, const int* snapshot_iters_host, int n_snap,
                                    const int* smooth_host, int n_smooth, float* out_fields, void* workspace, size_t workspace_bytes,
                                    void* stream);

int cvx_register_pairs_f32(int n_pairs, const float* const* img_fixed, const float* const* img_moving,
                           const float* const* feat_fixed, const float* const* feat_moving, const cvx_pair_params* p,
                           float* const* out_fields, int* out_dims_host, void* workspace, size_t workspace_bytes,
                           int n_streams, void* stream);

int cvx_last_pair_profile(const char** names_host, float* ms_host, int max_stages);
void cvx_set_profiling(int mode);

int cvx_jacobian_det_f32(const float* flow, int H, int W, int D, int convert1, float* out, void* stream);
int cvx_jacobian_stats_f64(const float* jac, int64_t n, double* acc3, void* stream);
int cvx_warp_labels_nearest_f32(const float* seg, const float* disp, int H, int W, int D, const float* base_h,
                                const float* base_w, const float* base_d, float* out, void* stream);
int cvx_label_overlap_i64(const float* a, const float* b, int64_t n, int num_labels, int64_t* counts, void* stream);
int cvx_map_coordinates_linear_f64(const double* moving, const double* disp, int H, int W, int D, double* out, void* stream);

size_t cvx_feature_transform_workspace_bytes(int H, int W, int D);
int cvx_feature_transform_i32(const float* obj, int H, int W, int D, int* feat, void* workspace, size_t workspace_bytes,
                              void* stream);
int cvx_feature_flat_index_i64(const int* feat, int H, int W, int D, int W_full, int D_full, int64_t* out, void* stream);

int cvx_label_mask_f32(const float* seg, int H, int W, int D, int label, int precision, float* inside, float* outside,
                       int64_t* count, void* stream);
int cvx_label_mask_scaled_f32(const float* seg, int H, int W, int D, int label, int Ho, int Wo, int Do, float scale_inv, float* inside,
                              float* outside, int64_t* count, void* stream);
int cvx_edt_sqdist_i32(const float* obj, const int* feat, int H, int W, int D, int* d2, void* stream);
int cvx_surface_hist_i64(const int* a_in2, const int* a_out2, const int* b_in2, int64_t n, int nbins, int64_t* hist, int* overflow,
                         void* stream);
int cvx_hist_order_stats_i64(const int64_t* hist, int nbins, int64_t k0, int64_t k1, int64_t* out3, void* stream);
int cvx_hist_percentile_neighbours_i64(const int64_t* hist, int nbins, float quantile, int64_t* out3, void* stream);
int cvx_surface_hist_batch_i64(const void* const* volumes_dev, int n_hist, int64_t n, int nbins, int64_t* hist, int* overflow, void* stream);
int cvx_hist_percentile_neighbours_batch_i64(const int64_t* hist, int nbins, int n_hist, float quantile, int64_t* out3, void* stream);
size_t cvx_edt_squared_workspace_bytes(int batch, int H, int W, int D);
int cvx_edt_squared_i32(const float* obj, int batch, int H, int W, int D, int* d2, void* workspace, size_t workspace_bytes,
                        void* stream);
int cvx_edt_squared_labels_i32(const float* seg, int H, int W, int D, const int* labels_host, int n_labels, int* d2, void* workspace,
                               size_t workspace_bytes, void* stream);
size_t cvx_label_bits_bytes(int H, int W, int D, int num_labels);
int cvx_label_bits_u64(const float* seg, int H, int W, int D, int num_labels, uint64_t* bits, void* stream);
int cvx_surface_distance_hist_i64(const float* seg_b, const uint64_t* bits_a, int H, int W, int D, int num_labels, const uint64_t* active4,
                                  int nbins, int64_t* hist, int64_t hist_stride, int* overflow, int overflow_stride, int max_radius, void* stream);
size_t cvx_surface_distance_hist_bits_workspace_bytes(int H, int W, int D, int num_labels);
int cvx_surface_distance_hist_bits_i64(const uint64_t* bits_b, const uint64_t* bits_a, int H, int W, int D, int num_labels,
                                       const uint64_t* active4, int nbins, int64_t* hist, int64_t hist_stride, int* overflow,
                                       int overflow_stride, int max_radius, void* workspace, size_t workspace_bytes, void* stream);

size_t cvx_tps_fit_workspace_bytes(int n, int nrhs);
int cvx_tps_fit_f32(const float* centres, const float* values, int n, int nrhs, float lambd, float* theta, void* workspace,
                    size_t workspace_bytes, void* stream);
int cvx_tps_eval_f32(const float* points, int64_t m, const float* centres, const float* theta, int n, int nrhs, float* out, void* stream);
int cvx_tps_dense_f32(int s0, int s1, int s2, const float* centres, const float* theta, int n, int nrhs, float* out, void* stream);
int cvx_resize_trilinear_ac_f32(const float* in, int C, int h, int w, int d, float* out, int H, int W, int D, void* stream);

#pragma GCC visibility pop

#ifdef __cplusplus
}
#endif
#endif
```

Measured before the change: 145.5.

## Pre-divide adjoint box taps in warp-gradient kernel; add optional flag-based tile sync

Moves the backward box filter's initial divide-by-27 pre-scaling into the warp-gradient store (on by default through CVX_BOX_PREDIV), so the tiled backward box kernel skips that prep step. This removes per-tap arithmetic from the box tile's first pass at the cost of a divide in warp_grad. It also adds an opt-in mode that replaces the workgroup barriers between the three box passes with per-row flags and spin-waits, plus timestamp census instrumentation and a sync-error counter. The flag mode is off by default and risks spin-wait timeouts if enabled.

Result: faster. 147.7, median of 6 (+1.5%).

```diff
diff --git a/convexadam_amd/_lib.py b/convexadam_amd/_lib.py
--- a/convexadam_amd/_lib.py
+++ b/convexadam_amd/_lib.py
@@ -50,6 +50,7 @@
     "cvx_set_mind_exp_table": (_i, [_vp, C.c_uint, C.c_uint]),
     "cvx_expf_f32": (_i, [_vp, _vp, _sz, _vp]),
     "cvx_set_option": (_i, [C.c_char_p, C.c_longlong]),
+    "cvx_box_tile_sync_errors": (_i, [_i]),
     "cvx_get_option": (C.c_longlong, [C.c_char_p]),
     "cvx_affine_base_host": (None, [_i, _vp]),
     "cvx_disp_mesh_host": (None, [_i, _vp]),
diff --git a/convexadam_amd/csrc/adam.hip b/convexadam_amd/csrc/adam.hip
--- a/convexadam_amd/csrc/adam.hip
+++ b/convexadam_amd/csrc/adam.hip
@@ -124,14 +124,21 @@
     v[i] = vv;
 }
 
+static int box3_tile_choice(const float* in, const float* out, int h, int w, int d, bool backward, const float* P, const float* m, const float* v,
+                            const float* gsave) {
+    if (options().box_tiled != 0) return 0;
+    if (!(backward ? (out || P) && box3_tile_supported(in, out, h, w, d, P, m, v, gsave) : box3_tile_fwd_supported(in, out, h, w, d))) return 0;
+    long long ft = backward ? options().box_bwd_tile : options().box_fwd_tile;
+    if (ft < 0) ft = box3_march_supported(d) ? box3_tile_fwd_auto(h, w, d) : 2000;
+    return ft >= 1000 ? (int)ft : 0;
+}
+
 static int launch_box3x3(const float* in, float* out, int h, int w, int d, bool backward, float* P, float* m, float* v,
-                         AdamConsts ac, float* gsave, hipStream_t s) {
+                         AdamConsts ac, float* gsave, bool prediv, hipStream_t s) {
+    const int ft = box3_tile_choice(in, out, h, w, d, backward, P, m, v, gsave);
+    if (ft) return launch_box3_tile(in, out, h, w, d, ft, backward, P, m, v, ac, gsave, prediv, s);
+    if (prediv) return fail(CVX_ERR_INVALID_ARG, "box3x3: pre-divided adjoint taps without the tile kernel");
     const bool force_tiled = options().box_tiled != 0;
-    if (!force_tiled && (backward ? (out || P) && box3_tile_supported(in, out, h, w, d, P, m, v, gsave) : box3_tile_fwd_supported(in, out, h, w, d))) {
-        long long ft = backward ? options().box_bwd_tile : options().box_fwd_tile;
-        if (ft < 0) ft = box3_march_supported(d) ? box3_tile_fwd_auto(h, w, d) : 2000;
-        if (ft >= 1000) return launch_box3_tile(in, out, h, w, d, (int)ft, backward, P, m, v, ac, gsave, s);
-    }
     if (!force_tiled && box3_march_supported(d)) return launch_box3_march(in, out, h, w, d, backward, P, m, v, ac, gsave, s);
     const int nb = cdiv(d, BT_X) * cdiv(w, BT_Y) * cdiv(h, BT_Z) * 3;
     if (!backward) hipLaunchKernelGGL((k_box3x3<false, false>), dim3(nb), dim3(BT_NT), 0, s, in, out, h, w, d, P, m, v, ac, gsave);
@@ -265,7 +272,7 @@
         const AdamConsts ac = {(float)(1.0 - beta1), (float)beta2, (float)(1.0 - beta2), (float)sqrt(bc2), (float)(-(1.0 / bc1)), adam_sqrt_table()};
         if (fast == 2 && fused) { if ((rc = launch_box3_fast(P, U, h, w, d, nullptr, nullptr, nullptr, 1.0, 1.0, nullptr, s))) return rc; }
         else if (fast == 2 && sm->kind == 0) { if ((rc = launch_boxchain_fast(P, U, h, w, d, *sm, false, s))) return rc; }
-        else if (fused) { if ((rc = launch_box3x3(P, U, h, w, d, false, nullptr, nullptr, nullptr, ac, nullptr, s))) return rc; }
+        else if (fused) { if ((rc = launch_box3x3(P, U, h, w, d, false, nullptr, nullptr, nullptr, ac, nullptr, false, s))) return rc; }
         else if ((rc = launch_smoother(P, U, t1, 3, h, w, d, *sm, false, s))) return rc;
         profile_mark_kernel("adam.forward_boxes", s);
         const bool last = it == niter - 1;
@@ -282,9 +289,10 @@
                 if (gsave) (void)hipMemcpyAsync(gsave, t2, sizeof(float) * 3 * V, hipMemcpyDeviceToDevice, s);
             }
         } else {
-        if ((rc = launch_warp_grad(Fcl, Mcl, C, h, w, d, U, base_h, base_w, base_d, gsc, cH, cW, cD, gU, f16_features, s))) return rc;
+        const bool prediv = fused && options().box_prediv != 0 && box3_tile_choice(gU, nullptr, h, w, d, true, P, m, v, gsave) != 0;
+        if ((rc = launch_warp_grad(Fcl, Mcl, C, h, w, d, U, base_h, base_w, base_d, gsc, cH, cW, cD, gU, f16_features, prediv, s))) return rc;
         profile_mark_kernel("adam.warp_gradient", s);
-        if (fused) { if ((rc = launch_box3x3(gU, nullptr, h, w, d, true, P, m, v, ac, gsave, s))) return rc; }
+        if (fused) { if ((rc = launch_box3x3(gU, nullptr, h, w, d, true, P, m, v, ac, gsave, prediv, s))) return rc; }
         else {
             if ((rc = launch_smoother(gU, t2, t1, 3, h, w, d, *sm, true, s))) return rc;
             hipLaunchKernelGGL(k_adam_update, dim3((unsigned)cdiv64((int64_t)(3 * V), 256)), dim3(256), 0, s, t2, P, m, v, 3 * V, ac);
diff --git a/convexadam_amd/csrc/api.hip b/convexadam_amd/csrc/api.hip
--- a/convexadam_amd/csrc/api.hip
+++ b/convexadam_amd/csrc/api.hip
@@ -47,7 +47,7 @@
             env_ll("CVX_NO_PRUNE", 0),     env_ll("CVX_CORR_UNFUSED", 0), env_ll("CVX_CORR_FUSED_ALL", 0), env_ll("CVX_PRUNE_STREAM_ABOVE", -1), env_ll("CVX_CF_CENSUS", 0), env_ll("CVX_CF_PRIO", 136),
             env_ll("CVX_WARP_FLAT", 0),    env_ll("CVX_BOX_YT", 8),       env_ll("CVX_BOX_WG_TARGET", 0),
             env_ll("CVX_BOX_XSPLIT", -1),  env_ll("CVX_BOX_CPT", 4),      env_ll("CVX_BOX_UNEVEN", 200), env_ll("CVX_BOX_ADAM_ROLE", 0), env_ll("CVX_BOX_DPP", 0),      env_ll("CVX_BOX_PK", 0),       env_ll("CVX_BOX_PRIO", 0),     env_ll("CVX_LABEL_POW_BLOCK", 32), 0,                             env_ll("CVX_MIND_MEAN_THREADS", 0),
-            env_ll("CVX_EDT_SEQUENTIAL", 0), env_ll("CVX_WARP_OCTANT", 4), env_ll("CVX_BOX_FWD_TILE", -1), env_ll("CVX_BOX_BWD_TILE", -1), env_ll("CVX_BOX_WALK", 1), env_ll("CVX_CORR_DUAL", 0), env_ll("CVX_PRUNE_REFINE", 1), env_ll("CVX_MIND_RECORDS", 1), env_ll("CVX_RESIZE_UP2", 1), env_ll("CVX_MIND_BLOCKED", 1), env_ll("CVX_CORR_CERT", 1), env_ll("CVX_CC_DEBUG", 0), env_ll("CVX_IC_FUSED", 0), env_ll("CVX_MIND_SINGLE", 0), env_ll("CVX_MS_ZLEN", 0), env_ll("CVX_CF_MAP", 1), env_ll("CVX_CERT_UNFUSED", 0), env_ll("CVX_FBOX_TILE", 0)};
+            env_ll("CVX_EDT_SEQUENTIAL", 0), env_ll("CVX_WARP_OCTANT", 4), env_ll("CVX_BOX_FWD_TILE", -1), env_ll("CVX_BOX_BWD_TILE", -1), env_ll("CVX_BOX_WALK", 1), env_ll("CVX_CORR_DUAL", 0), env_ll("CVX_PRUNE_REFINE", 1), env_ll("CVX_MIND_RECORDS", 1), env_ll("CVX_RESIZE_UP2", 1), env_ll("CVX_MIND_BLOCKED", 1), env_ll("CVX_CORR_CERT", 1), env_ll("CVX_CC_DEBUG", 0), env_ll("CVX_IC_FUSED", 0), env_ll("CVX_MIND_SINGLE", 0), env_ll("CVX_MS_ZLEN", 0), env_ll("CVX_CF_MAP", 1), env_ll("CVX_CERT_UNFUSED", 0), env_ll("CVX_FBOX_TILE", 0), env_ll("CVX_BOX_TILE_SYNC", 0), env_ll("CVX_BOX_PREDIV", 1), 0};
 }
 static cvx_context& default_context() {
     static cvx_context c = [] { cvx_context d; d.opt = env_options(); return d; }();
@@ -109,7 +109,7 @@
                                     {"prune_stream_above", &Options::prune_stream_above}, {"cf_census", &Options::cf_census}, {"cf_prio", &Options::cf_prio},
                                     {"warp_flat", &Options::warp_flat},       {"box_yt", &Options::box_yt},             {"box_wg_target", &Options::box_wg_target},
                                     {"box_xsplit", &Options::box_xsplit},     {"box_cpt", &Options::box_cpt},           {"box_uneven", &Options::box_uneven},     {"box_adam_role", &Options::box_adam_role}, {"box_dpp", &Options::box_dpp},           {"box_pk", &Options::box_pk},             {"box_prio", &Options::box_prio},         {"label_pow_block", &Options::label_pow_block}, {"census_ptr", &Options::census_ptr},     {"mind_mean_threads", &Options::mind_mean_threads},
-                                    {"edt_sequential", &Options::edt_sequential}, {"warp_octant", &Options::warp_octant}, {"box_fwd_tile", &Options::box_fwd_tile}, {"box_bwd_tile", &Options::box_bwd_tile}, {"box_walk", &Options::box_walk}, {"corr_dual", &Options::corr_dual}, {"prune_refine", &Options::prune_refine}, {"mind_records", &Options::mind_records}, {"resize_up2", &Options::resize_up2}, {"mind_blocked", &Options::mind_blocked}, {"corr_cert", &Options::corr_cert}, {"cc_debug", &Options::cc_debug}, {"ic_fused", &Options::ic_fused}, {"mind_single", &Options::mind_single}, {"ms_zlen", &Options::ms_zlen}, {"cf_map", &Options::cf_map}, {"cert_unfused", &Options::cert_unfused}, {"fbox_tile", &Options::fbox_tile}};
+                                    {"edt_sequential", &Options::edt_sequential}, {"warp_octant", &Options::warp_octant}, {"box_fwd_tile", &Options::box_fwd_tile}, {"box_bwd_tile", &Options::box_bwd_tile}, {"box_walk", &Options::box_walk}, {"corr_dual", &Options::corr_dual}, {"prune_refine", &Options::prune_refine}, {"mind_records", &Options::mind_records}, {"resize_up2", &Options::resize_up2}, {"mind_blocked", &Options::mind_blocked}, {"corr_cert", &Options::corr_cert}, {"cc_debug", &Options::cc_debug}, {"ic_fused", &Options::ic_fused}, {"mind_single", &Options::mind_single}, {"ms_zlen", &Options::ms_zlen}, {"cf_map", &Options::cf_map}, {"cert_unfused", &Options::cert_unfused}, {"fbox_tile", &Options::fbox_tile}, {"box_tile_sync", &Options::box_tile_sync}, {"box_prediv", &Options::box_prediv}, {"tile_census_ptr", &Options::tile_census_ptr}};
 
 }
 
diff --git a/convexadam_amd/csrc/boxtile.hip b/convexadam_amd/csrc/boxtile.hip
--- a/convexadam_amd/csrc/boxtile.hip
+++ b/convexadam_amd/csrc/boxtile.hip
@@ -71,18 +71,53 @@
     }
 }
 
-}
-
-template <int TZ, int TY, int TXQ, int NW, int WPS, bool BACKWARD, bool ADAM>
+constexpr unsigned BT_SPIN_MAX = 1u << 20;
+__device__ unsigned bt_sync_errors;
+
+__device__ __forceinline__ void bt_publish(int* flag, bool leader) {
+#ifdef CVX_RACE_JITTER
+    cvx_jitter();
+#endif
+    __builtin_amdgcn_fence(__ATOMIC_RELEASE, "workgroup");
+    if (leader) __hip_atomic_store(flag, 1, __ATOMIC_RELAXED, __HIP_MEMORY_SCOPE_WORKGROUP);
+}
+
+__device__ __forceinline__ void bt_wait(const int* flags, int Y, int planes, int ns, FastDiv dn, int r, int a, int b, int q) {
+#ifdef CVX_RACE_JITTER
+    cvx_jitter();
+#endif
+    for (unsigned spin = 0;; ++spin) {
+        bool ok = true;
+        if (q < 15)
+            for (int sg = q / 3; sg < ns; sg += 5)
+                if (fastdiv(sg * planes, dn) < b && fastdiv((sg + 1) * planes, dn) > a)
+                    ok = ok && __hip_atomic_load(flags + sg * Y + r + q % 3, __ATOMIC_RELAXED, __HIP_MEMORY_SCOPE_WORKGROUP) != 0;
+        if (__builtin_amdgcn_ballot_w64(!ok) == 0) break;
+        if (spin >= BT_SPIN_MAX) {
+            if (q == 0) atomicAdd(&bt_sync_errors, 1u);
+            break;
+        }
+        __builtin_amdgcn_s_sleep(1);
+    }
+    __builtin_amdgcn_fence(__ATOMIC_ACQUIRE, "workgroup");
+}
+
+}
+
+template <int TZ, int TY, int TXQ, int NW, int WPS, bool BACKWARD, bool ADAM, bool PREDIV, bool SYNC>
 __global__ __launch_bounds__(64 * NW, WPS) void k_box3_tile(const float* __restrict__ in, float* __restrict__ out, int h, int w, int d,
                                                            int ntz, int nty, int ntx, int ntiles, int NS1, int NS2, int NS3, FastDiv dvz, FastDiv dvx, FastDiv dvy,
                                                            FastDiv dn1, FastDiv dn2, FastDiv dn3, float* __restrict__ P, float* __restrict__ m, float* __restrict__ v, AdamConsts ac,
-                                                           float* __restrict__ gsave) {
+                                                           float* __restrict__ gsave, unsigned long long* __restrict__ census) {
     constexpr int TX = 4 * TXQ, RS = TX + 4;
     constexpr int Z1 = TZ + 4, Y1 = TY + 4, Z2 = TZ + 2, Y2 = TY + 2;
     constexpr int SLOTS = NW * 4;
+    constexpr int NF1 = Z1 / 2 * Y1, NF2 = Z2 / 2 * Y2;
     static_assert(TXQ + 2 <= 16, "a row of quads must fit 16 lanes");
     __shared__ __attribute__((aligned(16))) float S[Z1 * Y1 * RS + Z2 * Y2 * RS + 8];
+    __shared__ int RF[SYNC ? NF1 + NF2 : 1];
+    int* F1 = RF;
+    int* F2 = RF + NF1;
     float* S1 = S;
     float* S2 = S + Z1 * Y1 * RS;
     const int per_xcd = (int)(gridDim.x >> 3);
@@ -98,6 +133,13 @@
     const __amdgpu_buffer_rsrc_t ir = __builtin_amdgcn_make_buffer_rsrc(const_cast<float*>(ic), 0, (int)(V * sizeof(float)), 0x00020000);
     const int tid = threadIdx.x, q = tid & 15, slot = tid >> 4;
     const int wd = w * d;
+    if (SYNC) {
+        for (int i = tid; i < NF1 + NF2; i += 64 * NW) RF[i] = 0;
+        cvx_barrier();
+    }
+    unsigned long long* cw = (census && b < 1024) ? census + ((size_t)b * NW + __builtin_amdgcn_readfirstlane(tid >> 6)) * 8 : nullptr;
+    auto stamp = [&](int k) { if (cw && (tid & 63) == 0) cw[k] = __builtin_amdgcn_s_memrealtime(); };
+    stamp(0);
 
     for (int item = slot; item < Y1 * NS1; item += SLOTS) {
         const int r = item % Y1, sg = item / Y1;
@@ -122,7 +164,7 @@
             }
         };
         auto prep = [&](BTWin& t) {
-            if (BACKWARD) {
+            if (BACKWARD && !PREDIV) {
 #pragma unroll
                 for (int i = 0; i < 3; ++i)
 #pragma unroll
@@ -147,12 +189,18 @@
             if (q < TXQ + 1) lds_store2(p + 2, f32x2{o[2], o[3]});
         };
         bt_walk(L, load, prep, emit);
-    }
-    cvx_barrier();
+        if (SYNC) bt_publish(F1 + sg * Y1 + r, q == 0);
+    }
+    stamp(1);
+    if (!SYNC) { cvx_barrier(); stamp(2); }
 
     for (int item = slot; item < Y2 * NS2; item += SLOTS) {
         const int r = item % Y2, sg = item / Y2;
         const int p0 = fastdiv(sg * Z2, dn2), L = fastdiv((sg + 1) * Z2, dn2) - p0;
+        if (SYNC) {
+            bt_wait(F1, Y1, Z1, NS1, dn1, r, p0, p0 + L + 2, q);
+            if (item == slot) stamp(2);
+        }
         if (q < TXQ + 1) {
             const float* src = S1 + (p0 * Y1 + r) * RS + 4 * q;
             auto load = [&](int n, BTWin& t) {
@@ -182,12 +230,18 @@
             };
             bt_walk(L, load, [](BTWin&) {}, emit);
         }
-    }
-    cvx_barrier();
+        if (SYNC) bt_publish(F2 + sg * Y2 + r, q == 0);
+    }
+    stamp(3);
+    if (!SYNC) { cvx_barrier(); stamp(4); }
 
     for (int item = slot; item < TY * NS3; item += SLOTS) {
         const int r = item % TY, sg = item / TY;
         const int p0 = fastdiv(sg * TZ, dn3), L = fastdiv((sg + 1) * TZ, dn3) - p0;
+        if (SYNC) {
+            bt_wait(F2, Y2, Z2, NS2, dn2, r, p0, p0 + L + 2, q);
+            if (item == slot) stamp(4);
+        }
         const int gy = y0 + r, gx = x0 + 4 * q;
         if (q < TXQ && gy < w && gx < d) {
             const float* src = S2 + (p0 * Y2 + r) * RS + 4 * q;
@@ -223,6 +277,11 @@
             bt_walk(L, load, [](BTWin&) {}, emit);
         }
     }
+    stamp(5);
+    if (cw && (tid & 63) == 0) {
+        cw[6] = 0;
+        cw[7] = __builtin_amdgcn_s_getreg((4 << 0) | (0 << 6) | (31 << 11)) | ((unsigned long long)__builtin_amdgcn_s_getreg((20 << 0) | (0 << 6) | (31 << 11)) << 32);
+    }
 }
 
 bool box3_tile_supported(const float* in, const float* out, int h, int w, int d, const float* P, const float* m, const float* v, const float* gsave) {
@@ -233,33 +292,40 @@
 
 template <int TZ, int TY, int TXQ, int NW, int WPS>
 static int launch_tile_t(const float* in, float* out, int h, int w, int d, int ns1, int ns2, int ns3, bool backward, float* P, float* m, float* v,
-                         AdamConsts ac, float* gsave, hipStream_t s) {
+                         AdamConsts ac, float* gsave, bool prediv, hipStream_t s) {
     const int ntz = cdiv(h, TZ), nty = cdiv(w, TY), ntx = cdiv(d, 4 * TXQ);
     const int ntiles = 3 * ntz * nty * ntx;
     const unsigned nb = (unsigned)((ntiles + 7) / 8 * 8);
     auto clampns = [](int ns, int planes) { return ns < 1 ? 1 : (ns > planes / 2 ? planes / 2 : ns); };
     const int a1 = clampns(ns1, TZ + 4), a2 = clampns(ns2, TZ + 2), a3 = clampns(ns3, TZ);
-#define CVX_BT_LAUNCH(B, A) hipLaunchKernelGGL((k_box3_tile<TZ, TY, TXQ, NW, WPS, B, A>), dim3(nb), dim3(64 * NW), 0, s, in, out, h, w, d, ntz, nty, ntx, ntiles, a1, a2, a3, fastdiv_make(ntz), fastdiv_make(ntx), fastdiv_make(nty), fastdiv_make(a1), fastdiv_make(a2), fastdiv_make(a3), P, m, v, ac, gsave)
-    if (!backward) CVX_BT_LAUNCH(false, false);
-    else if (!P) CVX_BT_LAUNCH(true, false);
-    else CVX_BT_LAUNCH(true, true);
+    const bool sync = options().box_tile_sync != 0;
+    unsigned long long* census = reinterpret_cast<unsigned long long*>(options().tile_census_ptr);
+    if (census && backward) census += 8 * 16 * 1024;
+#define CVX_BT_LAUNCH(B, A, D, Y) hipLaunchKernelGGL((k_box3_tile<TZ, TY, TXQ, NW, WPS, B, A, D, Y>), dim3(nb), dim3(64 * NW), 0, s, in, out, h, w, d, ntz, nty, ntx, ntiles, a1, a2, a3, fastdiv_make(ntz), fastdiv_make(ntx), fastdiv_make(nty), fastdiv_make(a1), fastdiv_make(a2), fastdiv_make(a3), P, m, v, ac, gsave, census)
+#define CVX_BT_SYNC(B, A, D) do { if (sync) CVX_BT_LAUNCH(B, A, D, true); else CVX_BT_LAUNCH(B, A, D, false); } while (0)
+    if (!backward) CVX_BT_SYNC(false, false, false);
+    else if (!P) { if (prediv) CVX_BT_SYNC(true, false, true); else CVX_BT_SYNC(true, false, false); }
+    else if (prediv) CVX_BT_SYNC(true, true, true);
+    else CVX_BT_SYNC(true, true, false);
+#undef CVX_BT_SYNC
 #undef CVX_BT_LAUNCH
     return check_last("box3_tile");
 }
 
 int launch_box3_tile(const float* in, float* out, int h, int w, int d, int variant, bool backward, float* P, float* m, float* v, AdamConsts ac,
-                     float* gsave, hipStream_t s) {
+                     float* gsave, bool prediv, hipStream_t s) {
     const int kind = variant / 1000, ns = variant % 1000;
     int ns1 = ns / 100, ns2 = (ns / 10) % 10, ns3 = ns % 10;
+    prediv = prediv && backward;
     if (kind == 1) {
         if (!ns) { ns1 = 5; ns2 = 3; ns3 = 4; }
-        return launch_tile_t<12, 8, 14, 8, 4>(in, out, h, w, d, ns1, ns2, ns3, backward, P, m, v, ac, gsave, s);
+        return launch_tile_t<12, 8, 14, 8, 4>(in, out, h, w, d, ns1, ns2, ns3, backward, P, m, v, ac, gsave, prediv, s);
     }
     if (!ns) { ns1 = 4; ns2 = 3; ns3 = 4; }
-    return launch_tile_t<12, 16, 14, 16, 4>(in, out, h, w, d, ns1, ns2, ns3, backward, P, m, v, ac, gsave, s);
+    return launch_tile_t<12, 16, 14, 16, 4>(in, out, h, w, d, ns1, ns2, ns3, backward, P, m, v, ac, gsave, prediv, s);
 }
 int launch_box3_tile_fwd(const float* in, float* out, int h, int w, int d, int variant, hipStream_t s) {
-    return launch_box3_tile(in, out, h, w, d, variant, false, nullptr, nullptr, nullptr, AdamConsts{}, nullptr, s);
+    return launch_box3_tile(in, out, h, w, d, variant, false, nullptr, nullptr, nullptr, AdamConsts{}, nullptr, false, s);
 }
 
 int box3_tile_fwd_auto(int h, int w, int d) {
@@ -268,3 +334,13 @@
 }
 
 }
+
+extern "C" int cvx_box_tile_sync_errors(int reset) {
+    unsigned n = 0;
+    if (hipDeviceSynchronize() != hipSuccess || hipMemcpyFromSymbol(&n, HIP_SYMBOL(cvx::bt_sync_errors), sizeof(n)) != hipSuccess) return CVX_ERR_LAUNCH;
+    if (reset && n) {
+        const unsigned z = 0;
+        if (hipMemcpyToSymbol(HIP_SYMBOL(cvx::bt_sync_errors), &z, sizeof(z)) != hipSuccess || hipDeviceSynchronize() != hipSuccess) return CVX_ERR_LAUNCH;
+    }
+    return (int)n;
+}
diff --git a/convexadam_amd/csrc/cvx_common.h b/convexadam_amd/csrc/cvx_common.h
--- a/convexadam_amd/csrc/cvx_common.h
+++ b/convexadam_amd/csrc/cvx_common.h
@@ -92,6 +92,9 @@
     long long cf_map;
     long long cert_unfused;
     long long fbox_tile;
+    long long box_tile_sync;
+    long long box_prediv;
+    long long tile_census_ptr;
 };
 Options& options();
 const unsigned* adam_sqrt_table();
@@ -353,10 +356,10 @@
 int box3_tile_fwd_auto(int h, int w, int d);
 bool box3_tile_supported(const float* in, const float* out, int h, int w, int d, const float* P, const float* m, const float* v, const float* gsave);
 int launch_box3_tile(const float* in, float* out, int h, int w, int d, int variant, bool backward, float* P, float* m, float* v, AdamConsts ac,
-                     float* gsave, hipStream_t s);
+                     float* gsave, bool prediv, hipStream_t s);
 int launch_to_chunked(const float* in, int C, size_t V, float* out, bool half, hipStream_t s);
 int launch_warp_grad(const float* Fcl, const float* Mcl, int C, int h, int w, int d, const float* U, const float* bh,
-                     const float* bw, const float* bd, float gsc, float cH, float cW, float cD, float* gU, bool half, hipStream_t s);
+                     const float* bw, const float* bd, float gsc, float cH, float cW, float cD, float* gU, bool half, bool prediv, hipStream_t s);
 int launch_warp_grad_fast(const float* Fcl, const float* Mcl, int C, int h, int w, int d, const float* U, const float* bh,
                           const float* bw, const float* bd, float gsc, float cH, float cW, float cD, float* gU, bool half, hipStream_t s);
 int launch_box3_fast(const float* in, float* out, int h, int w, int d, float* P, float* m, float* v, double bc1, double bc2,
diff --git a/convexadam_amd/csrc/warp.hip b/convexadam_amd/csrc/warp.hip
--- a/convexadam_amd/csrc/warp.hip
+++ b/convexadam_amd/csrc/warp.hip
@@ -38,7 +38,7 @@
     return make_float4((float)v.x, (float)v.y, (float)v.z, (float)v.w);
 }
 
-template <bool BUF, bool HALF = false>
+template <bool BUF, bool HALF = false, bool PREDIV = false>
 __global__ __launch_bounds__(256) void k_warp_grad(const float* __restrict__ F2, const float* __restrict__ M2, int C, int CP,
                                                    int h, int w, int d, const float* __restrict__ U,
                                                    const float* __restrict__ bh, const float* __restrict__ bw,
@@ -137,7 +137,7 @@
         t = acc +  (cH * (2.0f * (uc - nb[a][3]))); acc = z > 0 ? t : acc;
         t = acc + -(cW * (2.0f * (nb[a][4] - uc))); acc = y < w - 1 ? t : acc;
         t = acc +  (cW * (2.0f * (uc - nb[a][5]))); acc = y > 0 ? t : acc;
-        (gU + (size_t)a * V)[p] = acc;
+        (gU + (size_t)a * V)[p] = PREDIV ? (acc == 0.0f ? acc : div_exact<27>(acc)) : acc;
     }
     if (census && threadIdx.x == 0) census[4 * blockIdx.x + 2] = __builtin_amdgcn_s_memrealtime();
 }
@@ -152,16 +152,19 @@
 }
 
 int launch_warp_grad(const float* Fcl, const float* Mcl, int C, int h, int w, int d, const float* U, const float* bh,
-                     const float* bw, const float* bd, float gsc, float cH, float cW, float cD, float* gU, bool half, hipStream_t s) {
+                     const float* bw, const float* bd, float gsc, float cH, float cW, float cD, float* gU, bool half, bool prediv, hipStream_t s) {
     const int CP = (C + 3) / 4 * 4;
     const dim3 gv((unsigned)((cdiv(d, 16) * cdiv(w, 4) * cdiv(h, 4) + 7) / 8 * 8));
     unsigned long long* census = reinterpret_cast<unsigned long long*>(options().census_ptr);
     if (census) census += 8 * 1024;
     const FastDiv dx = fastdiv_make(cdiv(d, 16)), dy = fastdiv_make(cdiv(w, 4));
     const float sc0 = (float)((h - 1) / 2.0), sc1 = (float)((w - 1) / 2.0), sc2 = (float)((d - 1) / 2.0);
-    if (half) hipLaunchKernelGGL((k_warp_grad<true, true>), gv, dim3(256), 0, s, Fcl, Mcl, C, CP, h, w, d, U, bh, bw, bd, gsc, cH, cW, cD, gU, census, dx, dy, sc0, sc1, sc2);
-    else if (options().warp_flat) hipLaunchKernelGGL(k_warp_grad<false>, gv, dim3(256), 0, s, Fcl, Mcl, C, CP, h, w, d, U, bh, bw, bd, gsc, cH, cW, cD, gU, census, dx, dy, sc0, sc1, sc2);
-    else hipLaunchKernelGGL(k_warp_grad<true>, gv, dim3(256), 0, s, Fcl, Mcl, C, CP, h, w, d, U, bh, bw, bd, gsc, cH, cW, cD, gU, census, dx, dy, sc0, sc1, sc2);
+#define CVX_WG_LAUNCH(...) hipLaunchKernelGGL((k_warp_grad<__VA_ARGS__>), gv, dim3(256), 0, s, Fcl, Mcl, C, CP, h, w, d, U, bh, bw, bd, gsc, cH, cW, cD, gU, census, dx, dy, sc0, sc1, sc2)
+    if (half) { if (prediv) CVX_WG_LAUNCH(true, true, true); else CVX_WG_LAUNCH(true, true); }
+    else if (options().warp_flat) { if (prediv) CVX_WG_LAUNCH(false, false, true); else CVX_WG_LAUNCH(false); }
+    else if (prediv) CVX_WG_LAUNCH(true, false, true);
+    else CVX_WG_LAUNCH(true);
+#undef CVX_WG_LAUNCH
     return check_last("warp_grad");
 }
 
diff --git a/include/convexadam_hip.h b/include/convexadam_hip.h
--- a/include/convexadam_hip.h
+++ b/include/convexadam_hip.h
@@ -30,6 +30,7 @@
 long long cvx_context_get_option(const cvx_context* ctx, const char* name);
 int cvx_set_option(const char* name, long long value);
 long long cvx_get_option(const char* name);
+int cvx_box_tile_sync_errors(int reset);
 
 void cvx_affine_base_host(int S, float* out_host);
 void cvx_disp_mesh_host(int disp_hw, float* out_host);
```
